# RLinf/RLinf

Measured on NVIDIA H100. Metric: env-steps/sec (rollout+update), higher is better.
Workload: dtype f32

## Files before the change

### include/rlinf_b200.h

```cpp
#ifndef RLINF_B200_H
#define RLINF_B200_H

#include <stdint.h>

#ifdef __cplusplus
extern "C" {
#endif

#define RB200_ABI_VERSION 2

#define RB200_OK 0
#define RB200_E_NULL (-1)
#define RB200_E_SHAPE (-2)
#define RB200_E_ARG (-3)
#define RB200_E_ALIGN (-4)
#define RB200_E_UNSUPPORTED (-5)

typedef void* rb200_stream_t;

int rb200_abi_version(void);
const char* rb200_strerror(int code);
int rb200_device_info(int* sm_count, int* cc_major, int* cc_minor);
uint64_t rb200_launch_count(void);

int rb200_loss_mask(const uint8_t* dones, uint8_t* mask, int64_t* mask_sum,
                    int nc, int B, int C, rb200_stream_t stream);

int rb200_gae(const float* rewards, const float* values, const uint8_t* dones,
              const uint8_t* loss_mask, float* adv, float* ret, double* stats,
              int T, int B, double gamma, double gae_lambda, rb200_stream_t stream);

int rb200_normalize(float* x, const double* stats, int64_t n_elems, float eps,
                    rb200_stream_t stream);

int rb200_grpo_scores(const float* rewards, const uint8_t* dones, float* scores,
                      int T, int B, rb200_stream_t stream);
int rb200_grpo_advantages(const float* scores, const uint8_t* loss_mask, float* adv,
                          int T, int B, int G, float eps, rb200_stream_t stream);

int rb200_gather_rows(const void* src, const int64_t* idx, void* dst, int64_t n_rows_out,
                      int64_t n_rows_src, int64_t row_bytes, rb200_stream_t stream);

enum { RB200_LOGPROB_TOKEN = 0, RB200_LOGPROB_ACTION = 1, RB200_LOGPROB_CHUNK = 2 };

enum {
  RB200_M_POLICY_LOSS = 0,
  RB200_M_POLICY_LOSS_ABS = 1,
  RB200_M_RATIO = 2,
  RB200_M_RATIO_ABS = 3,
  RB200_M_CLIPPED_RATIO = 4,
  RB200_M_DUAL_CLIPPED_RATIO = 5,
  RB200_M_APPROX_KL = 6,
  RB200_M_CLIP_FRACTION = 7,
  RB200_M_VALUE_LOSS = 8,
  RB200_M_VALUE_CLIP_RATIO = 9,
  RB200_M_EV_COUNT = 10,
  RB200_M_EV_RET_SUM = 11,
  RB200_M_EV_RET_SQ_SUM = 12,
  RB200_M_EV_ERR_SUM = 13,
  RB200_M_EV_ERR_SQ_SUM = 14,
  RB200_M_ENTROPY = 15,
  RB200_M_TOTAL_LOSS = 16,
  RB200_M_TOKEN_NUM = 17,
  RB200_NUM_METRICS = 24
};

typedef struct rb200_ppo_args {
  int64_t bsz;
  int32_t C, A;
  int32_t logprob_type;
  int32_t with_critic;
  const float* logprobs;
  const float* values;
  const float* entropy;
  const int64_t* idx;
  const float* old_logprobs;
  const float* advantages;
  const float* returns;
  const float* prev_values;
  const uint8_t* loss_mask;
  const int64_t* loss_mask_sum;
  int64_t mask_sum_row_mod;
  const double* adv_stats;
  float adv_norm_eps;
  double clip_ratio_low, clip_ratio_high;
  double clip_ratio_c;
  int32_t has_clip_log_ratio_min, has_clip_log_ratio_max;
  double clip_log_ratio_min, clip_log_ratio_max;
  double value_clip, huber_delta;
  int32_t max_episode_steps;
  int32_t critic_warmup;
  double entropy_bonus;
  double loss_scale;
  double* workspace;
  float* loss;
  float* metrics;
  float* d_logprobs;
  float* d_values;
  float* d_entropy;
} rb200_ppo_args;

int rb200_ppo_loss(const rb200_ppo_args* args, rb200_stream_t stream);

enum {
  RB200_DM_POLICY_LOSS = 0,
  RB200_DM_PROXIMAL_RATIO = 1,
  RB200_DM_CLIPPED_PROXIMAL_RATIO = 2,
  RB200_DM_CLIP_FRACTION = 3,
  RB200_DM_DUAL_CLIP_FRACTION = 4,
  RB200_DM_BEHAV_CLIP_FRACTION = 5,
  RB200_DM_PROXIMAL_APPROX_KL = 6,
  RB200_DM_BEHAV_APPROX_KL = 7,
  RB200_DM_VALUE_LOSS = 8,
  RB200_DM_VALUE_CLIP_RATIO = 9,
  RB200_DM_EV_COUNT = 10,
  RB200_DM_AVERAGE_VERSION = 15,
  RB200_DM_TOTAL_LOSS = 16,
  RB200_DM_TOKEN_NUM = 17,
  RB200_DM_CURRENT_VERSION = 18,
  RB200_DM_HAS_VERSION_METRICS = 19,
  RB200_DM_ENTROPY = 20
};
typedef struct rb200_dppo_args {
  rb200_ppo_args base;
  const float* proximal_logprobs;
  const float* versions;
  int32_t has_current_version;
  double current_version;
  int32_t has_behave_weight_threshold;
  double behave_weight_threshold;
} rb200_dppo_args;
int rb200_decoupled_ppo_loss(const rb200_dppo_args* args, rb200_stream_t stream);

typedef struct rb200_dppo_scalar_version_args {
  rb200_ppo_args base;
  const float* proximal_logprobs;
  double version;
  double current_version;
  int32_t has_behave_weight_threshold;
  double behave_weight_threshold;
} rb200_dppo_scalar_version_args;
int rb200_decoupled_ppo_loss_scalar_version(const rb200_dppo_scalar_version_args* args, rb200_stream_t stream);

enum { RB200_OM_POLICY_LOSS = 0, RB200_OM_OPD_REWARD = 1, RB200_OM_OPD_REVERSE_KL = 2, RB200_OM_TOTAL_LOSS = 16 };
int rb200_opd_loss(const float* logprobs, const float* advantages, const uint8_t* loss_mask,
                   const int64_t* loss_mask_sum, int64_t n_units, int tokens_per_unit, int max_episode_steps,
                   double loss_scale, double* workspace, float* loss ,
                   float* metrics , float* d_logprobs , rb200_stream_t stream);

enum { RB200_AGG_TOKEN_MEAN = 0, RB200_AGG_SEQ_MEAN_TOKEN_SUM = 1, RB200_AGG_SEQ_MEAN_TOKEN_MEAN = 2 };
enum {
  RB200_TM_POLICY_LOSS = 0,
  RB200_TM_POLICY_LOSS_ABS = 1,
  RB200_TM_RATIO = 2,
  RB200_TM_RATIO_ABS = 3,
  RB200_TM_CLIPPED_RATIO = 4,
  RB200_TM_DUAL_CLIPPED_RATIO = 5,
  RB200_TM_APPROX_KL = 6,
  RB200_TM_CLIP_FRACTION = 7,
  RB200_TM_ENTROPY_LOSS = 8,
  RB200_TM_KL_LOSS = 9,
  RB200_TM_FINAL_LOSS = 10,
  RB200_TM_ROLLOUT_TRAIN_KL = 11,
  RB200_TM_NUM = 16
};
typedef struct rb200_token_loss_args {
  int64_t bsz, L;
  const float* logprobs;            int64_t logprobs_stride;
  const float* old_logprobs;        int64_t old_logprobs_stride;
  const float* advantages;          int64_t advantages_stride;
  const uint8_t* loss_mask;         int64_t loss_mask_stride;
  const float* entropy;             int64_t entropy_stride;
  const float* ref_logprobs;        int64_t ref_logprobs_stride;
  const float* rollout_logprobs;    int64_t rollout_logprobs_stride;
  const float* recomputed_logprobs; int64_t recomputed_logprobs_stride;
  double clip_ratio_low, clip_ratio_high;
  double clip_ratio_c;
  double clip_log_ratio_min, clip_log_ratio_max;
  double entropy_bonus, kl_beta, importance_sampling_clip;
  int32_t has_clip_log_ratio_min, has_clip_log_ratio_max;
  int32_t agg;
  int32_t kl_mode;
  int32_t kl_order;
  int32_t importance_sampling_fix;
  int32_t fast_path_zero_loss_mask;
  int32_t reserved;
  void* workspace;
  int64_t workspace_bytes;
  float* loss;
  float* metrics;
  float* d_logprobs;
  float* d_entropy;
} rb200_token_loss_args;
int64_t rb200_token_loss_workspace_bytes(int64_t bsz, int64_t L);
int rb200_token_ppo_loss(const rb200_token_loss_args* args, rb200_stream_t stream);

enum {
  RB200_CM_VALUE_LOSS = 0,
  RB200_CM_VALUE_CLIP_RATIO = 1,
  RB200_CM_EV_COUNT = 2,
  RB200_CM_EV_RET_SUM = 3,
  RB200_CM_EV_RET_SQ_SUM = 4,
  RB200_CM_EV_ERR_SUM = 5,
  RB200_CM_EV_ERR_SQ_SUM = 6,
  RB200_CM_FINAL_VALUE_LOSS = 7,
  RB200_CM_NUM = 8
};
typedef struct rb200_token_critic_loss_args {
  int64_t bsz, L;
  const float* values;       int64_t values_stride;
  const float* returns;      int64_t returns_stride;
  const float* prev_values;  int64_t prev_values_stride;
  const uint8_t* loss_mask;  int64_t loss_mask_stride;
  double value_clip, huber_delta;
  void* workspace;
  int64_t workspace_bytes;
  float* loss;
  float* metrics;
  float* d_values;
} rb200_token_critic_loss_args;
int rb200_token_critic_loss(const rb200_token_critic_loss_args* args, rb200_stream_t stream);

int64_t rb200_value_head_workspace_bytes(int64_t n, int64_t H);
int rb200_value_head_fwd(const void* x, int64_t row_stride, const int64_t* rows, int64_t n, int64_t H, const void* w,
                         float* v, rb200_stream_t stream);
int rb200_value_head_bwd(const void* x, int64_t row_stride, const int64_t* rows, int64_t n, int64_t H, const float* g,
                         const void* w, const int64_t* inv_map, int64_t T, void* dx, void* dw, void* workspace,
                         int64_t workspace_bytes, rb200_stream_t stream);

int rb200_scale(float* x, int64_t n, float s, rb200_stream_t stream);
int rb200_scale_by(float* x, int64_t n, const float* s_dev, rb200_stream_t stream);

int rb200_grad_sqnorm(const float* grads, int64_t n, double* out_sq ,
                      rb200_stream_t stream);
int rb200_adamw_step(float* params, const float* grads, float* exp_avg, float* exp_avg_sq,
                     int64_t n, const int64_t* group_end_host, const double* group_lr_host,
                     int n_groups, double beta1, double beta2, double eps, double weight_decay,
                     float max_grad_norm, float grad_scale, const double* grad_sq ,
                     double* state , rb200_stream_t stream);
int rb200_adamw_step_dev(float* params, const float* grads, float* exp_avg, float* exp_avg_sq,
                         int64_t n, const int64_t* group_end_host, const double* group_lr_dev,
                         int n_groups, double beta1, double beta2, double eps, double weight_decay,
                         float max_grad_norm, float grad_scale, const double* grad_sq ,
                         double* state , rb200_stream_t stream);


typedef struct rb200_mlp_layout {
  int32_t obs_dim, act_dim , value_dim, hidden ;
  int64_t logstd;
  int64_t vw0, vb0, vw1, vb1, vw2, vb2, vw3;
  int64_t bw0, bb0, bw1, bb1, bw2, bb2;
  int64_t mw, mb;
  int64_t total;
} rb200_mlp_layout;

int rb200_mlp_layout_init(rb200_mlp_layout* L, int obs_dim, int act_dim, int value_dim, int hidden);

int64_t rb200_mlp_fwd_scratch_floats(const rb200_mlp_layout* L, int64_t n);

int64_t rb200_mlp_wsplit_floats(const rb200_mlp_layout* L);
int rb200_mlp_prepare_weights(const rb200_mlp_layout* L, const float* params, float* wsplit,
                              rb200_stream_t stream);

int rb200_mlp_forward(const rb200_mlp_layout* L, const float* params, const float* wsplit,
                      const float* states, const float* action, const int64_t* idx, int64_t n,
                      float* logprobs, float* entropy, float* values, float* acts, float* work,
                      const float* states_amax, rb200_stream_t stream);
int rb200_absmax(const float* x, int64_t rows, int cols, float* out, rb200_stream_t stream);

int rb200_mlp_backward(const rb200_mlp_layout* L, const float* params, const float* wsplit,
                       const float* states, const float* action, const int64_t* idx, int64_t n,
                       const float* d_logprobs, const float* d_entropy, const float* d_values,
                       const float* acts, float* work, float* grads, rb200_stream_t stream);

int rb200_mlp_sample(const rb200_mlp_layout* L, const float* params, const float* wsplit,
                     const float* states, const float* noise, uint64_t seed, uint64_t offset,
                     const uint64_t* counter_dev, int64_t n, float* action, float* logprobs, float* values,
                     float* work, rb200_stream_t stream);

int rb200_tc_gemm_h(const float* A, const float* B, float* C, int64_t M, int K, int mode, const float* amax,
                    float* work, rb200_stream_t stream);
int rb200_tc_wgrad_h(const float* Z, const float* H, float* dW, int64_t n, int IN, const float* amax,
                     rb200_stream_t stream);
int rb200_tc_dgrad_wgrad_h(const float* Z, const float* W, const float* H, float* dZprev, float* dW, float* colsum,
                           const float* amax_in, float* amax_out, int64_t n, int ngroups, float* work,
                           rb200_stream_t stream);

int rb200_debug_set_flags(int flags);

typedef struct rb200_rollout_args {
  float* states;
  float* actions;
  float* logprobs;
  float* values;
  float* rewards;
  uint8_t* terminations;
  uint8_t* truncations;
  uint8_t* dones;
  float* final_obs;
  float* final_values;
  const float* w_s;
  const float* w_a;
  int32_t* elapsed;
  const float* policy_noise;
  const float* env_noise;
  const uint64_t* counter_policy;
  const uint64_t* counter_env;
  float* episode_return;
  double* episode_acc;
  uint64_t seed_policy, seed_env, offset_policy;
  int32_t T, B;
  int32_t num_action_chunks;
  int32_t max_episode_steps, auto_reset;
  int32_t bootstrap_on_done;
  double gamma, p_term, noise_std, reward_noise_std;
} rb200_rollout_args;

int64_t rb200_rollout_fused_wt_floats(const rb200_mlp_layout* L);
int rb200_rollout_fused_supported(const rb200_mlp_layout* L, int B);
int rb200_rollout_fused_prepare(const rb200_mlp_layout* L, const float* params, float* wt, rb200_stream_t stream);
int rb200_rollout_fused(const rb200_mlp_layout* L, const float* params, const float* wt, const rb200_rollout_args* a,
                        rb200_stream_t stream);

int rb200_rollout_tc_supported(const rb200_mlp_layout* L, int num_action_chunks, int B);
int64_t rb200_rollout_tc_pack_bytes(const rb200_mlp_layout* L);
int rb200_rollout_tc_prepare(const rb200_mlp_layout* L, const float* params, const float* w_s, void* pack,
                             rb200_stream_t stream);
int rb200_rollout_tc(const rb200_mlp_layout* L, const float* params, const void* pack, const rb200_rollout_args* a,
                     rb200_stream_t stream);

int rb200_logits_logprob_entropy_fwd(const void* logits, int dtype, const int64_t* target, int64_t N, int64_t L,
                                     int64_t batch_stride, int64_t row_stride, int V, int v_lo, int v_hi,
                                     double inv_temperature, float* logprob, float* entropy, float* lse,
                                     rb200_stream_t stream);
int rb200_logits_logprob_entropy_bwd(const void* logits, int dtype, const int64_t* target, int64_t N, int64_t L,
                                     int64_t batch_stride, int64_t row_stride, int V, int v_lo, int v_hi,
                                     double inv_temperature, const float* lse, const float* entropy,
                                     const float* grad_logprob, const float* grad_entropy, void* dlogits,
                                     int64_t d_batch_stride, int64_t d_row_stride, rb200_stream_t stream);

int64_t rb200_lmhead_workspace_bytes(int64_t N, int64_t L, int H, int V, int v_lo, int v_hi, int64_t vocab_chunk);
int rb200_lmhead_logprob_entropy_fwd(const void* hidden, const void* weight, const int64_t* target, int64_t N, int64_t L,
                                     int64_t batch_stride, int64_t row_stride, int H, int V, int v_lo, int v_hi,
                                     double inv_temperature, float* logprob, float* entropy, float* lse,
                                     void* workspace, int64_t workspace_bytes, rb200_stream_t stream);
int rb200_lmhead_logprob_entropy_bwd(const void* hidden, const void* weight, const int64_t* target, int64_t N, int64_t L,
                                     int64_t batch_stride, int64_t row_stride, int H, int V, int v_lo, int v_hi,
                                     double inv_temperature, const float* lse, const float* entropy,
                                     const float* grad_logprob, const float* grad_entropy, void* d_hidden,
                                     void* d_weight, void* workspace, int64_t workspace_bytes, rb200_stream_t stream);

int64_t rb200_lmhead_vp_workspace_bytes(int64_t N, int64_t L, int H, int Vs, int64_t vocab_start, int v_lo, int v_hi,
                                        int64_t vocab_chunk);
int rb200_lmhead_vp_partials_fwd(const void* hidden, const void* weight_shard, const int64_t* target, int64_t N,
                                 int64_t L, int64_t batch_stride, int64_t row_stride, int H, int Vs,
                                 int64_t vocab_start, int v_lo, int v_hi, double inv_temperature, float* record,
                                 void* workspace, int64_t workspace_bytes, rb200_stream_t stream);
int rb200_lmhead_vp_logprob_entropy_bwd(const void* hidden, const void* weight_shard, const int64_t* target,
                                        int64_t N, int64_t L, int64_t batch_stride, int64_t row_stride, int H, int Vs,
                                        int64_t vocab_start, int v_lo, int v_hi, double inv_temperature,
                                        const float* lse, const float* entropy, const float* grad_logprob,
                                        const float* grad_entropy, float* d_hidden_partial, void* d_weight_shard,
                                        void* workspace, int64_t workspace_bytes, rb200_stream_t stream);
int rb200_logits_vp_partials_fwd(const void* logits, int dtype, const int64_t* target, int64_t N, int64_t L,
                                 int64_t batch_stride, int64_t row_stride, int Vs, int64_t vocab_start, int v_lo,
                                 int v_hi, double inv_temperature, float* record, rb200_stream_t stream);
int rb200_vp_combine(const float* records, int n_ranks, int64_t N, const int64_t* target, int vocab_shard, int v_lo,
                     int v_hi, float* logprob, float* entropy, float* lse, rb200_stream_t stream);

enum {
  RB200_RR_RESPONSE = 1,
  RB200_RR_PROMPT = 2,
  RB200_RR_BOUNDS = 4,
  RB200_RR_ORDER = 8,
  RB200_RR_MAX_PROMPT = 16,
  RB200_RR_CAPACITY = 32
};
int rb200_response_rows_plan(int layout, const int64_t* len0, const int64_t* len1, const int64_t* response_lengths,
                             int64_t bsz, int64_t S, int64_t L, int64_t T, int entropy_shift, const int64_t* tokens,
                             int64_t capacity, int64_t* rows, int64_t* targets, int64_t* cell_map,
                             int64_t* hidden_map, int64_t* cells, int64_t* status, rb200_stream_t stream);

enum {
  RB200_RR_SHARD = 64,
  RB200_RR_CP_ALIGN = 128
};
int rb200_response_rows_mp_plan(const int64_t* cu_seqlens_padded, const int64_t* seq_lengths,
                                const int64_t* response_lengths, const int64_t* responses, int64_t bsz, int64_t L,
                                int64_t T_c, int tp_size, int cp_size, int sequence_parallel, int tp_rank, int cp_rank,
                                int64_t capacity_c, int64_t capacity_k, int64_t* rows, int64_t* send, int64_t* unpad,
                                int64_t* slot_map, int64_t* targets, int64_t* cell_map, int64_t* cells,
                                int64_t* hidden_map, int64_t* status, rb200_stream_t stream);
int rb200_response_rows_mp_pack_grad(const float* dx, const int64_t* idx, void* out, int64_t n_out, int64_t H,
                                     rb200_stream_t stream);

int rb200_mlp_value(const rb200_mlp_layout* L, const float* params, const float* wsplit,
                    const float* states, int64_t n, float* values, float* work, rb200_stream_t stream);

int rb200_synth_env_step(const float* w_s, const float* w_a, const float* state, const float* action,
                         const float* noise, float* next_state, float* final_obs, float* reward,
                         uint8_t* term, uint8_t* trunc, uint8_t* done, int32_t* elapsed, float* z_scratch,
                         int B, int obs, int act, int max_episode_steps, int auto_reset, float p_term,
                         float noise_std, float reward_noise_std, uint64_t seed,
                         const uint64_t* counter_dev, rb200_stream_t stream);
int rb200_synth_env_chunk_step(const float* w_s, const float* w_a, const float* state, const float* chunk_actions,
                               const float* noise, float* next_state, float* final_obs, float* rewards,
                               uint8_t* term, uint8_t* trunc, uint8_t* done, int32_t* elapsed, float* scratch,
                               int B, int obs, int act, int C, int max_episode_steps, int auto_reset, float p_term,
                               float noise_std, float reward_noise_std, uint64_t seed, const uint64_t* counter_dev,
                               rb200_stream_t stream);
int rb200_bootstrap_rewards_ld(float* rewards, int ld_rewards, const float* final_values, int value_dim,
                               const uint8_t* flag, int ld_flag, int B, double gamma, rb200_stream_t stream);
int rb200_bootstrap_rewards(float* rewards, const float* final_values, const uint8_t* flag, int B,
                            int value_dim, double gamma, rb200_stream_t stream);
int rb200_counter_add(uint64_t* counter_dev, uint64_t inc, rb200_stream_t stream);

int rb200_mlp_mean(const rb200_mlp_layout* L, const float* params, const float* wsplit, const float* states,
                   int64_t n, float* action, float* logprobs, float* values, float* work, rb200_stream_t stream);
int rb200_episode_stats_step(const float* rewards, const uint8_t* done, int B, int C, int auto_reset, float* ret,
                             int32_t* len, uint8_t* prev_done, double* acc, float* episode, rb200_stream_t stream);
int rb200_episode_stats_reduce(const double* acc, int B, double* out, rb200_stream_t stream);
int rb200_train_episode_stats_step(const float* rewards, const uint8_t* done, int B, int C, int auto_reset,
                                   int last_step, float* ret, int32_t* len, double* acc, rb200_stream_t stream);

int rb200_reward_filter(const float* rewards, const uint8_t* loss_mask, uint8_t* out_mask, uint8_t* keep_env,
                        int nc, int B, int C, int group_size, float lower, float upper,
                        rb200_stream_t stream);

int rb200_kl_penalty(const float* logprob, const float* ref_logprob, float* out, float* d_logprob, int64_t n,
                     int mode, rb200_stream_t stream);

int rb200_masked_stats(const float* x, const uint8_t* mask, int64_t n, int64_t mask_div, double* out4,
                       rb200_stream_t stream);

int rb200_masked_moments(const float* x, const uint8_t* mask, int64_t n, double* out3 ,
                         rb200_stream_t stream);
int rb200_masked_normalize(const float* x, const uint8_t* mask, float* out, int64_t n, const double* stats3,
                           int mode, double eps, int unbiased, rb200_stream_t stream);
int rb200_raw_advantages(const float* scores , const uint8_t* loss_mask , float* adv ,
                         int L, int B, double* stats3, rb200_stream_t stream);
int rb200_reinpp_returns(const float* rewards , const uint8_t* loss_mask , const float* logprob,
                         const float* ref_logprob, float* ret , int L, int B, double kl_beta, int kl_mode,
                         double* stats3, rb200_stream_t stream);
int rb200_grpo_video_advantages(const float* rewards , const float* mask_f32, const uint8_t* mask_u8,
                                float* adv , int S, int B, int G, int mode, float eps, rb200_stream_t stream);
int rb200_grpo_dynamic_turn_advantages(const float* rewards , const int32_t* idx_to_traj ,
                                       float* turn_adv , int n, int num_trajectories, int G, int mode,
                                       float eps, rb200_stream_t stream);
int rb200_sub(const float* a, const float* b, float* out, int64_t n, rb200_stream_t stream);

#ifdef __cplusplus
}
#endif
#endif
```

### rlinf_b200/_lib.py

```python
from __future__ import annotations

import ctypes as C
import os
from typing import Optional

import torch

_PKG_DIR = os.path.dirname(os.path.abspath(__file__))
LIB_PATH = os.path.join(_PKG_DIR, "librlinf_b200.so")

c_void_p, c_int, c_int64, c_float, c_double, c_uint64 = C.c_void_p, C.c_int, C.c_int64, C.c_float, C.c_double, C.c_uint64

NUM_METRICS = 24
LOGPROB_TYPES = {"token_level": 0, "action_level": 1, "chunk_level": 2}

M_KEYS = {
    0: "actor/policy_loss", 1: "actor/policy_loss_abs", 2: "actor/ratio", 3: "actor/ratio_abs",
    4: "actor/clipped_ratio", 5: "actor/dual_cliped_ratio", 6: "actor/approx_kl", 7: "actor/clip_fraction",
    8: "critic/value_loss", 9: "critic/value_clip_ratio",
    10: "__sum__/_critic_explained_variance/count",
    11: "__sum__/_critic_explained_variance/returns_sum",
    12: "__sum__/_critic_explained_variance/returns_sq_sum",
    13: "__sum__/_critic_explained_variance/errors_sum",
    14: "__sum__/_critic_explained_variance/errors_sq_sum",
    15: "actor/entropy_loss", 16: "actor/total_loss", 17: "actor/token_num",
}
ACTOR_SLOTS = (0, 1, 2, 3, 4, 5, 6, 7)
CRITIC_SLOTS = (8, 9, 10, 11, 12, 13, 14)


class PpoArgs(C.Structure):
    _fields_ = [
        ("bsz", c_int64), ("C", C.c_int32), ("A", C.c_int32), ("logprob_type", C.c_int32), ("with_critic", C.c_int32),
        ("logprobs", c_void_p), ("values", c_void_p), ("entropy", c_void_p),
        ("idx", c_void_p), ("old_logprobs", c_void_p), ("advantages", c_void_p), ("returns", c_void_p),
        ("prev_values", c_void_p), ("loss_mask", c_void_p), ("loss_mask_sum", c_void_p),
        ("mask_sum_row_mod", c_int64),
        ("adv_stats", c_void_p), ("adv_norm_eps", c_float),
        ("clip_ratio_low", c_double), ("clip_ratio_high", c_double), ("clip_ratio_c", c_double),
        ("has_clip_log_ratio_min", C.c_int32), ("has_clip_log_ratio_max", C.c_int32),
        ("clip_log_ratio_min", c_double), ("clip_log_ratio_max", c_double),
        ("value_clip", c_double), ("huber_delta", c_double),
        ("max_episode_steps", C.c_int32), ("critic_warmup", C.c_int32),
        ("entropy_bonus", c_double), ("loss_scale", c_double),
        ("workspace", c_void_p),
        ("loss", c_void_p), ("metrics", c_void_p), ("d_logprobs", c_void_p), ("d_values", c_void_p),
        ("d_entropy", c_void_p),
    ]


class DppoArgs(C.Structure):
    _fields_ = [("base", PpoArgs), ("proximal_logprobs", c_void_p), ("versions", c_void_p),
                ("has_current_version", C.c_int32), ("current_version", c_double),
                ("has_behave_weight_threshold", C.c_int32), ("behave_weight_threshold", c_double)]


class DppoScalarVersionArgs(C.Structure):
    _fields_ = [("base", PpoArgs), ("proximal_logprobs", c_void_p), ("version", c_double),
                ("current_version", c_double), ("has_behave_weight_threshold", C.c_int32),
                ("behave_weight_threshold", c_double)]


class RolloutArgs(C.Structure):
    _fields_ = [(n, c_void_p) for n in (
        "states", "actions", "logprobs", "values", "rewards", "terminations", "truncations", "dones", "final_obs",
        "final_values", "w_s", "w_a", "elapsed", "policy_noise", "env_noise", "counter_policy", "counter_env",
        "episode_return", "episode_acc")] + [
        ("seed_policy", c_uint64), ("seed_env", c_uint64), ("offset_policy", c_uint64),
        ("T", C.c_int32), ("B", C.c_int32), ("num_action_chunks", C.c_int32), ("max_episode_steps", C.c_int32),
        ("auto_reset", C.c_int32), ("bootstrap_on_done", C.c_int32),
        ("gamma", c_double), ("p_term", c_double), ("noise_std", c_double), ("reward_noise_std", c_double),
    ]


DM_KEYS = {
    0: "actor/policy_loss", 1: "actor/proximal_ratio", 2: "actor/clipped_proximal_ratio", 3: "actor/clip_fraction",
    4: "actor/dual_clip_fraction", 5: "actor/behav_clip_fraction", 6: "actor/proximal_approx_kl",
    7: "actor/behav_approx_kl", 8: "critic/value_loss", 9: "critic/value_clip_ratio",
    10: "__sum__/_critic_explained_variance/count", 11: "__sum__/_critic_explained_variance/returns_sum",
    12: "__sum__/_critic_explained_variance/returns_sq_sum", 13: "__sum__/_critic_explained_variance/errors_sum",
    14: "__sum__/_critic_explained_variance/errors_sq_sum",
}
DM_ENTROPY = 20


AGG_MODES = {"token-mean": 0, "seq-mean-token-sum": 1, "seq-mean-token-mean": 2}
TM_NUM = 16
TM_KEYS = {
    0: "actor/policy_loss", 1: "actor/policy_loss_abs", 2: "actor/ratio", 3: "actor/ratio_abs",
    4: "actor/clipped_ratio", 5: "actor/dual_cliped_ratio", 6: "actor/approx_kl", 7: "actor/clip_fraction",
    8: "actor/entropy_loss", 9: "actor/kl_loss", 10: "actor/final_loss", 11: "actor/rollout_train_kl",
}


class TokenLossArgs(C.Structure):
    _fields_ = [("bsz", c_int64), ("L", c_int64)] + [
        f for name in ("logprobs", "old_logprobs", "advantages", "loss_mask", "entropy", "ref_logprobs",
                       "rollout_logprobs", "recomputed_logprobs") for f in ((name, c_void_p), (name + "_stride", c_int64))
    ] + [(n, c_double) for n in ("clip_ratio_low", "clip_ratio_high", "clip_ratio_c", "clip_log_ratio_min",
                                  "clip_log_ratio_max", "entropy_bonus", "kl_beta", "importance_sampling_clip")] + [
        (n, C.c_int32) for n in ("has_clip_log_ratio_min", "has_clip_log_ratio_max", "agg", "kl_mode", "kl_order",
                                 "importance_sampling_fix", "fast_path_zero_loss_mask", "reserved")] + [
        ("workspace", c_void_p), ("workspace_bytes", c_int64),
        ("loss", c_void_p), ("metrics", c_void_p), ("d_logprobs", c_void_p), ("d_entropy", c_void_p),
    ]


CM_NUM = 8
CM_KEYS = {
    0: "critic/value_loss", 1: "critic/value_clip_ratio",
    2: "__sum__/_critic_explained_variance/count",
    3: "__sum__/_critic_explained_variance/returns_sum",
    4: "__sum__/_critic_explained_variance/returns_sq_sum",
    5: "__sum__/_critic_explained_variance/errors_sum",
    6: "__sum__/_critic_explained_variance/errors_sq_sum",
    7: "critic/final_value_loss",
}


class TokenCriticLossArgs(C.Structure):
    _fields_ = [("bsz", c_int64), ("L", c_int64)] + [
        f for name in ("values", "returns", "prev_values", "loss_mask")
        for f in ((name, c_void_p), (name + "_stride", c_int64))
    ] + [("value_clip", c_double), ("huber_delta", c_double), ("workspace", c_void_p), ("workspace_bytes", c_int64),
         ("loss", c_void_p), ("metrics", c_void_p), ("d_values", c_void_p)]


class MlpLayout(C.Structure):
    _fields_ = [
        ("obs_dim", C.c_int32), ("act_dim", C.c_int32), ("value_dim", C.c_int32), ("hidden", C.c_int32),
        ("logstd", c_int64),
        ("vw0", c_int64), ("vb0", c_int64), ("vw1", c_int64), ("vb1", c_int64), ("vw2", c_int64), ("vb2", c_int64),
        ("vw3", c_int64),
        ("bw0", c_int64), ("bb0", c_int64), ("bw1", c_int64), ("bb1", c_int64), ("bw2", c_int64), ("bb2", c_int64),
        ("mw", c_int64), ("mb", c_int64), ("total", c_int64),
    ]


SIGNATURES = {
    "rb200_abi_version": (c_int, []),
    "rb200_strerror": (C.c_char_p, [c_int]),
    "rb200_device_info": (c_int, [C.POINTER(c_int)] * 3),
    "rb200_launch_count": (c_uint64, []),
    "rb200_loss_mask": (c_int, [c_void_p, c_void_p, c_void_p, c_int, c_int, c_int, c_void_p]),
    "rb200_gae": (c_int, [c_void_p] * 7 + [c_int, c_int, c_double, c_double, c_void_p]),
    "rb200_normalize": (c_int, [c_void_p, c_void_p, c_int64, c_float, c_void_p]),
    "rb200_grpo_scores": (c_int, [c_void_p, c_void_p, c_void_p, c_int, c_int, c_void_p]),
    "rb200_grpo_advantages": (c_int, [c_void_p, c_void_p, c_void_p, c_int, c_int, c_int, c_float, c_void_p]),
    "rb200_gather_rows": (c_int, [c_void_p, c_void_p, c_void_p, c_int64, c_int64, c_int64, c_void_p]),
    "rb200_ppo_loss": (c_int, [C.POINTER(PpoArgs), c_void_p]),
    "rb200_decoupled_ppo_loss": (c_int, [C.POINTER(DppoArgs), c_void_p]),
    "rb200_decoupled_ppo_loss_scalar_version": (c_int, [C.POINTER(DppoScalarVersionArgs), c_void_p]),
    "rb200_opd_loss": (c_int, [c_void_p] * 4 + [c_int64, c_int, c_int, c_double] + [c_void_p] * 5),
    "rb200_token_loss_workspace_bytes": (c_int64, [c_int64, c_int64]),
    "rb200_token_ppo_loss": (c_int, [C.POINTER(TokenLossArgs), c_void_p]),
    "rb200_scale": (c_int, [c_void_p, c_int64, c_float, c_void_p]),
    "rb200_scale_by": (c_int, [c_void_p, c_int64, c_void_p, c_void_p]),
    "rb200_grad_sqnorm": (c_int, [c_void_p, c_int64, c_void_p, c_void_p]),
    "rb200_adamw_step": (c_int, [c_void_p] * 4 + [c_int64, C.POINTER(c_int64), C.POINTER(c_double), c_int,
                                                  c_double, c_double, c_double, c_double, c_float, c_float,
                                                  c_void_p, c_void_p, c_void_p]),
    "rb200_adamw_step_dev": (c_int, [c_void_p] * 4 + [c_int64, C.POINTER(c_int64), c_void_p, c_int,
                                                      c_double, c_double, c_double, c_double, c_float, c_float,
                                                      c_void_p, c_void_p, c_void_p]),
    "rb200_mlp_layout_init": (c_int, [C.POINTER(MlpLayout), c_int, c_int, c_int, c_int]),
    "rb200_mlp_fwd_scratch_floats": (c_int64, [C.POINTER(MlpLayout), c_int64]),
    "rb200_mlp_wsplit_floats": (c_int64, [C.POINTER(MlpLayout)]),
    "rb200_mlp_prepare_weights": (c_int, [C.POINTER(MlpLayout), c_void_p, c_void_p, c_void_p]),
    "rb200_mlp_forward": (c_int, [C.POINTER(MlpLayout)] + [c_void_p] * 5 + [c_int64] + [c_void_p] * 7),
    "rb200_absmax": (c_int, [c_void_p, c_int64, c_int, c_void_p, c_void_p]),
    "rb200_mlp_backward": (c_int, [C.POINTER(MlpLayout)] + [c_void_p] * 5 + [c_int64] + [c_void_p] * 7),
    "rb200_mlp_sample": (c_int, [C.POINTER(MlpLayout)] + [c_void_p] * 4 + [c_uint64, c_uint64, c_void_p, c_int64] + [c_void_p] * 5),
    "rb200_tc_gemm_h": (c_int, [c_void_p, c_void_p, c_void_p, c_int64, c_int, c_int, c_void_p, c_void_p, c_void_p]),
    "rb200_tc_wgrad_h": (c_int, [c_void_p, c_void_p, c_void_p, c_int64, c_int, c_void_p, c_void_p]),
    "rb200_tc_dgrad_wgrad_h": (c_int, [c_void_p] * 8 + [c_int64, c_int, c_void_p, c_void_p]),
    "rb200_debug_set_flags": (c_int, [c_int]),
    "rb200_rollout_fused_wt_floats": (c_int64, [C.POINTER(MlpLayout)]),
    "rb200_rollout_fused_supported": (c_int, [C.POINTER(MlpLayout), c_int]),
    "rb200_rollout_fused_prepare": (c_int, [C.POINTER(MlpLayout), c_void_p, c_void_p, c_void_p]),
    "rb200_rollout_fused": (c_int, [C.POINTER(MlpLayout), c_void_p, c_void_p, C.POINTER(RolloutArgs), c_void_p]),
    "rb200_rollout_tc_supported": (c_int, [C.POINTER(MlpLayout), c_int, c_int]),
    "rb200_rollout_tc_pack_bytes": (c_int64, [C.POINTER(MlpLayout)]),
    "rb200_rollout_tc_prepare": (c_int, [C.POINTER(MlpLayout), c_void_p, c_void_p, c_void_p, c_void_p]),
    "rb200_rollout_tc": (c_int, [C.POINTER(MlpLayout), c_void_p, c_void_p, C.POINTER(RolloutArgs), c_void_p]),
    "rb200_logits_logprob_entropy_fwd": (c_int, [c_void_p, c_int, c_void_p, c_int64, c_int64, c_int64, c_int64, c_int,
                                                 c_int, c_int, c_double, c_void_p, c_void_p, c_void_p, c_void_p]),
    "rb200_logits_logprob_entropy_bwd": (c_int, [c_void_p, c_int, c_void_p, c_int64, c_int64, c_int64, c_int64, c_int,
                                                 c_int, c_int, c_double] + [c_void_p] * 5 + [c_int64, c_int64, c_void_p]),
    "rb200_lmhead_workspace_bytes": (c_int64, [c_int64, c_int64, c_int, c_int, c_int, c_int, c_int64]),
    "rb200_lmhead_logprob_entropy_fwd": (c_int, [c_void_p, c_void_p, c_void_p, c_int64, c_int64, c_int64, c_int64, c_int,
                                                 c_int, c_int, c_int, c_double] + [c_void_p] * 4 + [c_int64, c_void_p]),
    "rb200_lmhead_logprob_entropy_bwd": (c_int, [c_void_p, c_void_p, c_void_p, c_int64, c_int64, c_int64, c_int64, c_int,
                                                 c_int, c_int, c_int, c_double] + [c_void_p] * 7 + [c_int64, c_void_p]),
    "rb200_lmhead_vp_workspace_bytes": (c_int64, [c_int64, c_int64, c_int, c_int, c_int64, c_int, c_int, c_int64]),
    "rb200_lmhead_vp_partials_fwd": (c_int, [c_void_p, c_void_p, c_void_p, c_int64, c_int64, c_int64, c_int64, c_int,
                                             c_int, c_int64, c_int, c_int, c_double, c_void_p, c_void_p, c_int64,
                                             c_void_p]),
    "rb200_lmhead_vp_logprob_entropy_bwd": (c_int, [c_void_p, c_void_p, c_void_p, c_int64, c_int64, c_int64, c_int64,
                                                    c_int, c_int, c_int64, c_int, c_int, c_double] + [c_void_p] * 7
                                            + [c_int64, c_void_p]),
    "rb200_logits_vp_partials_fwd": (c_int, [c_void_p, c_int, c_void_p, c_int64, c_int64, c_int64, c_int64, c_int,
                                             c_int64, c_int, c_int, c_double, c_void_p, c_void_p]),
    "rb200_vp_combine": (c_int, [c_void_p, c_int, c_int64, c_void_p, c_int, c_int, c_int] + [c_void_p] * 4),
    "rb200_response_rows_plan": (c_int, [c_int, c_void_p, c_void_p, c_void_p, c_int64, c_int64, c_int64, c_int64,
                                         c_int, c_void_p, c_int64] + [c_void_p] * 6 + [c_void_p]),
    "rb200_response_rows_mp_plan": (c_int, [c_void_p] * 4 + [c_int64] * 3 + [c_int] * 5 + [c_int64] * 2
                                    + [c_void_p] * 9 + [c_void_p]),
    "rb200_response_rows_mp_pack_grad": (c_int, [c_void_p, c_void_p, c_void_p, c_int64, c_int64, c_void_p]),
    "rb200_token_critic_loss": (c_int, [C.POINTER(TokenCriticLossArgs), c_void_p]),
    "rb200_value_head_workspace_bytes": (c_int64, [c_int64, c_int64]),
    "rb200_value_head_fwd": (c_int, [c_void_p, c_int64, c_void_p, c_int64, c_int64, c_void_p, c_void_p, c_void_p]),
    "rb200_value_head_bwd": (c_int, [c_void_p, c_int64, c_void_p, c_int64, c_int64, c_void_p, c_void_p, c_void_p,
                                     c_int64, c_void_p, c_void_p, c_void_p, c_int64, c_void_p]),
    "rb200_mlp_value":(c_int, [C.POINTER(MlpLayout), c_void_p, c_void_p, c_void_p, c_int64, c_void_p, c_void_p, c_void_p]),
    "rb200_synth_env_step": (c_int, [c_void_p] * 13 + [c_int] * 5 + [c_float] * 3 + [c_uint64, c_void_p, c_void_p]),
    "rb200_synth_env_chunk_step": (c_int, [c_void_p] * 13 + [c_int] * 6 + [c_float] * 3 + [c_uint64, c_void_p, c_void_p]),
    "rb200_bootstrap_rewards_ld": (c_int, [c_void_p, c_int, c_void_p, c_int, c_void_p, c_int, c_int, c_double, c_void_p]),
    "rb200_bootstrap_rewards": (c_int, [c_void_p, c_void_p, c_void_p, c_int, c_int, c_double, c_void_p]),
    "rb200_reward_filter": (c_int, [c_void_p] * 4 + [c_int] * 4 + [c_float, c_float, c_void_p]),
    "rb200_kl_penalty": (c_int, [c_void_p] * 4 + [c_int64, c_int, c_void_p]),
    "rb200_masked_stats": (c_int, [c_void_p, c_void_p, c_int64, c_int64, c_void_p, c_void_p]),
    "rb200_counter_add": (c_int, [c_void_p, c_uint64, c_void_p]),
    "rb200_masked_moments": (c_int, [c_void_p, c_void_p, c_int64, c_void_p, c_void_p]),
    "rb200_masked_normalize": (c_int, [c_void_p, c_void_p, c_void_p, c_int64, c_void_p, c_int, c_double, c_int, c_void_p]),
    "rb200_raw_advantages": (c_int, [c_void_p, c_void_p, c_void_p, c_int, c_int, c_void_p, c_void_p]),
    "rb200_reinpp_returns": (c_int, [c_void_p] * 5 + [c_int, c_int, c_double, c_int, c_void_p, c_void_p]),
    "rb200_grpo_video_advantages": (c_int, [c_void_p] * 4 + [c_int, c_int, c_int, c_int, c_float, c_void_p]),
    "rb200_grpo_dynamic_turn_advantages": (c_int, [c_void_p] * 3 + [c_int, c_int, c_int, c_int, c_float, c_void_p]),
    "rb200_sub": (c_int, [c_void_p, c_void_p, c_void_p, c_int64, c_void_p]),
    "rb200_mlp_mean": (c_int, [C.POINTER(MlpLayout), c_void_p, c_void_p, c_void_p, c_int64] + [c_void_p] * 5),
    "rb200_episode_stats_step": (c_int, [c_void_p, c_void_p, c_int, c_int, c_int] + [c_void_p] * 6),
    "rb200_episode_stats_reduce": (c_int, [c_void_p, c_int, c_void_p, c_void_p]),
    "rb200_train_episode_stats_step": (c_int, [c_void_p, c_void_p] + [c_int] * 4 + [c_void_p] * 4),
}

_LIB: Optional[C.CDLL] = None


class Rb200Error(RuntimeError):
    pass


def load() -> C.CDLL:
    global _LIB
    if _LIB is not None:
        return _LIB
    if not os.path.exists(LIB_PATH):
        raise Rb200Error(
            f"{LIB_PATH} not found: build it with `python -m rlinf_b200.build` "
            "(nvcc, sm_90a). rlinf_b200 has no CPU or PyTorch fallback.")
    lib = C.CDLL(LIB_PATH)
    for name, (res, args) in SIGNATURES.items():
        fn = getattr(lib, name)
        fn.restype = res
        fn.argtypes = args
    _LIB = lib
    return lib


def check(code: int, what: str = "") -> None:
    if code == 0:
        return
    msg = load().rb200_strerror(code).decode()
    if code < 0:
        raise ValueError(f"rlinf_b200 {what}: {msg} (code {code})")
    raise Rb200Error(f"rlinf_b200 {what}: CUDA error {code}: {msg}")


def ptr(t: Optional[torch.Tensor]):
    if t is None:
        return None
    if not t.is_cuda:
        raise Rb200Error("rlinf_b200 kernels take CUDA tensors; move inputs with to_device() first")
    if not t.is_contiguous():
        raise Rb200Error("rlinf_b200 kernels take contiguous tensors")
    return c_void_p(t.data_ptr())


def stream_ptr(device=None):
    return c_void_p(torch.cuda.current_stream(device).cuda_stream)


def default_device() -> torch.device:
    if not torch.cuda.is_available():
        raise Rb200Error("rlinf_b200 needs a CUDA device (H100, sm_90a); there is no CPU fallback")
    return torch.device("cuda", torch.cuda.current_device())


def to_device(t: Optional[torch.Tensor], device=None, dtype=None) -> Optional[torch.Tensor]:
    if t is None:
        return None
    device = device or default_device()
    if t.device != device:
        t = t.to(device, non_blocking=True)
    if dtype is not None and t.dtype != dtype:
        t = t.to(dtype)
    return t.contiguous()


def as_u8(t: Optional[torch.Tensor]) -> Optional[torch.Tensor]:
    if t is None:
        return None
    if t.dtype == torch.bool:
        return t.view(torch.uint8)
    if t.dtype != torch.uint8:
        return (t != 0).view(torch.uint8)
    return t
```

### rlinf_b200/actor.py

```python
from __future__ import annotations

from typing import Optional

import numpy as np
import torch
import torch.distributed as dist

from . import _lib as L
from . import dist_utils as D
from . import ops
from .algorithms import calculate_adv_and_returns
from .config import wrap
from .lr_scheduler import LRSchedule
from .policy import FlatAdamW, MLPPolicy

EV_KEY = "critic/explained_variance"
_T_PLUS_ONE_KEYS = ("dones", "terminations", "truncations", "prev_values")


def process_nested_dict_for_adv(nested, rollout_epoch):
    out = {}
    for k, v in nested.items():
        if isinstance(v, dict):
            out[k] = process_nested_dict_for_adv(v, rollout_epoch)
        elif isinstance(v, torch.Tensor):
            x = v.reshape(rollout_epoch, -1, *v.shape[1:]).transpose(0, 1)
            out[k] = x.reshape(x.shape[0], -1, *x.shape[3:])
    return out


def process_nested_dict_for_train(nested, shuffle_id):
    out = {}
    for k, v in nested.items():
        if v is None:
            out[k] = None
        elif isinstance(v, dict):
            out[k] = process_nested_dict_for_train(v, shuffle_id)
        elif isinstance(v, torch.Tensor):
            if k in _T_PLUS_ONE_KEYS:
                v = v[:-1]
            flat = v.reshape(-1, *v.shape[2:])
            if any(s == 0 for s in flat.stride()) and flat.numel() > 1:
                flat = flat.contiguous()
            as_bool = flat.dtype == torch.bool
            src = flat.contiguous()
            res = ops.gather_rows(src.view(torch.uint8) if as_bool else src, shuffle_id)
            out[k] = res.view(torch.bool) if as_bool else res
    return out


class EmbodiedActor:
    def __init__(self, cfg, policy: Optional[MLPPolicy] = None, rank: Optional[int] = None,
                 world_size: Optional[int] = None, process_group=None):
        self.cfg = wrap(cfg)
        self.pg = process_group
        self._dist = dist.is_available() and dist.is_initialized()
        self._rank = rank if rank is not None else (dist.get_rank() if self._dist else 0)
        self._world_size = world_size if world_size is not None else (dist.get_world_size() if self._dist else 1)
        m = self.cfg.actor.model
        self.device = L.default_device()
        self.model = policy or MLPPolicy(m.obs_dim, m.action_dim, m.get("num_action_chunks", 1),
                                         add_value_head=m.get("add_value_head", True), device=self.device,
                                         seed=self.cfg.actor.seed)
        o = self.cfg.actor.optim
        self.optimizer = FlatAdamW(self.model, lr=o.lr, value_lr=o.get("value_lr", o.lr),
                                   betas=(o.get("adam_beta1", 0.9), o.get("adam_beta2", 0.999)),
                                   eps=o.get("adam_eps", 1e-8), weight_decay=o.get("weight_decay", 1e-2),
                                   clip_grad=o.get("clip_grad", 1.0))
        self.optimizer_steps = 0
        self.critic_warmup_steps = int(o.get("critic_warmup_steps", 0) or 0) if self.model.value_dim > 0 else 0
        self._with_critic = self.cfg.algorithm.adv_type == "gae"
        self._set_frozen_groups()
        self.lr_schedule = LRSchedule(o, base_lr=o.lr)
        self.optimizer.lr_scale = self.lr_schedule.multiplier()
        self.rollout_batch: dict = {}
        self._perm_cache: dict = {}
        self.version = 0
        self._graph_update = self.cfg.actor.get("cuda_graph_update", False)
        self._graph_multi_rank = bool(self.cfg.actor.get("cuda_graph_multi_rank", False))
        self._capture_nccl = bool(self.cfg.actor.get("cuda_graph_capture_nccl", True))
        self._static_batch: dict = {}
        self._step_graphs: dict = {}
        self._train_calls = 0
        self._states_amax = torch.zeros(4 + m.obs_dim if m.obs_dim <= 256 else 1, dtype=torch.float32,
                                        device=self.device) if m.obs_dim % 32 == 0 else None

    def recv_rollout_trajectories(self, batch: dict) -> None:
        def to_dev(d):
            return {k: (to_dev(v) if isinstance(v, dict) else L.to_device(v, self.device)) for k, v in d.items()
                    if v is not None}

        self.rollout_batch = self._process_received_rollout_batch(to_dev(batch))

    def _process_received_rollout_batch(self, rollout_batch: dict) -> dict:
        cfg = self.cfg
        rollout_epoch = cfg.env.train.get("rollout_epoch", 1)
        if rollout_epoch != 1:
            rollout_batch = process_nested_dict_for_adv(rollout_batch, rollout_epoch)
        if not cfg.env.train.auto_reset and not cfg.env.train.get("ignore_terminations", False):
            loss_mask, loss_mask_sum = ops.loss_mask(rollout_batch["dones"])
            if cfg.algorithm.reward_type == "chunk_level":
                loss_mask = loss_mask.any(dim=-1, keepdim=True)
                loss_mask_sum = loss_mask_sum[..., -1:]
            rollout_batch["loss_mask"] = loss_mask
            rollout_batch["loss_mask_sum"] = loss_mask_sum
        if cfg.algorithm.get("filter_rewards", False):
            rollout_batch["loss_mask"] = ops.reward_filter(
                rollout_batch["rewards"], rollout_batch.get("loss_mask", None), cfg.algorithm.group_size,
                cfg.algorithm.rewards_lower_bound, cfg.algorithm.rewards_upper_bound)
        return rollout_batch

    def compute_advantages_and_returns(self) -> dict:
        cfg, rb = self.cfg, self.rollout_batch
        kwargs = {
            "task_type": cfg.runner.task_type, "adv_type": cfg.algorithm.adv_type, "rewards": rb["rewards"],
            "dones": rb["dones"], "values": rb.get("prev_values", None), "prev_logprobs": rb.get("prev_logprobs", None),
            "teacher_logprobs": None, "num_action_chunks": cfg.actor.model.get("num_action_chunks", 1),
            "gamma": cfg.algorithm.get("gamma", 1), "gae_lambda": cfg.algorithm.get("gae_lambda", 1),
            "group_size": cfg.algorithm.get("group_size", 8), "reward_type": cfg.algorithm.reward_type,
            "loss_mask": rb.get("loss_mask", None), "loss_mask_sum": rb.get("loss_mask_sum", None),
            "advantage_mode": cfg.algorithm.get("advantage_mode", None),
        }
        rb.update(calculate_adv_and_returns(**kwargs))
        if not cfg.runner.get("rollout_metrics", True):
            return {}
        from .metric_utils import compute_rollout_metrics

        return compute_rollout_metrics(rb, self._world_size, self.pg)

    def _shuffle_id(self, n: int) -> torch.Tensor:
        key = (n, self.cfg.actor.seed + self._rank)
        if key not in self._perm_cache:
            g = torch.Generator()
            g.manual_seed(D.shuffle_seed(self.cfg.actor.seed, self._rank))
            self._perm_cache[key] = torch.randperm(n, generator=g).to(self.device)
        return self._perm_cache[key]

    def run_training(self) -> dict:
        cfg = self.cfg
        rb = self.rollout_batch
        rollout_size = rb["prev_logprobs"].shape[0] * rb["prev_logprobs"].shape[1]
        shuffle_id = self._shuffle_id(rollout_size)
        batch = process_nested_dict_for_train(rb, shuffle_id)
        self.rollout_batch = batch
        mbs = cfg.actor.micro_batch_size
        batch_size_per_rank, self.gradient_accumulation, n_global = D.per_rank_batch(
            cfg.actor.global_batch_size, self._world_size, mbs, rollout_size)
        update_epoch = cfg.algorithm.get("update_epoch", 1)
        n_steps = update_epoch * n_global
        n_micro = n_steps * self.gradient_accumulation
        metric_rows = torch.zeros(n_micro, L.NUM_METRICS, dtype=torch.float32, device=self.device)
        step_rows = torch.zeros(n_steps, 4, dtype=torch.float64, device=self.device)
        lr_rows = []
        mi = si = 0
        use_graph = self._graph_update
        if use_graph == "auto":
            use_graph = batch_size_per_rank <= 65536
        if self._world_size > 1 and not self._graph_multi_rank:
            use_graph = False
        graphed = bool(use_graph) and self._train_calls > 0
        self._train_calls += 1
        if graphed:
            batch = self._persist_batch(batch)
            self.rollout_batch = batch
        if self._states_amax is not None:
            ops.absmax(batch["forward_inputs"]["states"], out=self._states_amax)
        for _ in range(update_epoch):
            for gb in range(n_global):
                if graphed:
                    lr_rows.append(self._graphed_step(batch, gb, batch_size_per_rank, mbs,
                                                      metric_rows[mi: mi + self.gradient_accumulation], step_rows[si]))
                    mi += self.gradient_accumulation
                    si += 1
                    continue
                self.optimizer.zero_grad()
                for k in range(self.gradient_accumulation):
                    lo = gb * batch_size_per_rank + k * mbs
                    self.train_micro_batch(batch, lo, lo + mbs, metric_rows[mi])
                    mi += 1
                grad_norm_state, lr_list = self.optimizer_step()
                step_rows[si].copy_(grad_norm_state)
                lr_rows.append(lr_list)
                si += 1
        self.optimizer.lr_scale = self.lr_schedule.step()
        self.optimizer.zero_grad()
        return self._reduce_metrics(metric_rows, step_rows, lr_rows)

    def _persist_batch(self, batch: dict, prefix: str = "") -> dict:
        out = {}
        for k, v in batch.items():
            key = prefix + k
            if isinstance(v, dict):
                out[k] = self._persist_batch(v, key + "/")
            elif isinstance(v, torch.Tensor):
                buf = self._static_batch.get(key)
                if buf is None or buf.shape != v.shape or buf.dtype != v.dtype:
                    buf = torch.empty_like(v)
                    self._static_batch[key] = buf
                    self._step_graphs.clear()
                buf.copy_(v)
                out[k] = buf
            else:
                out[k] = v
        return out

    def _graphed_step(self, batch, gb, batch_size_per_rank, mbs, metric_out, state_out):
        warm = self.optimizer_steps < self.critic_warmup_steps
        accum = self.gradient_accumulation
        key = (gb, warm, accum, mbs, batch_size_per_rank, self._world_size)
        self.optimizer.sync_lr_table()
        entry = self._step_graphs.get(key)
        if entry is None:
            stage_m = torch.zeros(accum, L.NUM_METRICS, dtype=torch.float32, device=self.device)
            stage_s = torch.zeros(4, dtype=torch.float64, device=self.device)
            scale = 1.0 / self._world_size

            def fwd_bwd():
                self.optimizer.zero_grad()
                for k in range(accum):
                    lo = gb * batch_size_per_rank + k * mbs
                    self.train_micro_batch(batch, lo, lo + mbs, stage_m[k])

            def opt():
                self.optimizer.step(grad_scale=scale)
                stage_s.copy_(self.optimizer.state)

            graphs = None
            if self._world_size > 1 and self._capture_nccl:
                try:
                    torch.cuda.synchronize()
                    self.model.mark_params_changed()
                    g_all = torch.cuda.CUDAGraph()
                    with torch.cuda.graph(g_all):
                        fwd_bwd()
                        dist.all_reduce(self.model.flat_grads, op=dist.ReduceOp.SUM, group=self.pg)
                        opt()
                    graphs = (g_all, None)
                except Exception as e:
                    self._capture_nccl = False
                    self._capture_nccl_error = repr(e)
                    torch.cuda.synchronize()
            if graphs is None:
                torch.cuda.synchronize()
                self.model.mark_params_changed()
                g_a = torch.cuda.CUDAGraph()
                with torch.cuda.graph(g_a):
                    fwd_bwd()
                g_b = torch.cuda.CUDAGraph()
                with torch.cuda.graph(g_b, pool=g_a.pool()):
                    opt()
                graphs = (g_a, g_b)
            entry = (graphs, stage_m, stage_s)
            self._step_graphs[key] = entry
        (g_a, g_b), stage_m, stage_s = entry
        g_a.replay()
        self.optimizer_steps += 1
        if g_b is not None:
            D.allreduce_flat_grads(self.model.flat_grads, self._world_size, self.pg)
            g_b.replay()
        self.model.mark_params_changed()
        metric_out.copy_(stage_m)
        state_out.copy_(stage_s)
        return self._after_optimizer_step()

    def train_micro_batch(self, batch, lo, hi, metric_out) -> None:
        cfg = self.cfg
        fi = batch["forward_inputs"]
        with_critic = self._with_critic
        ent_bonus = float(cfg.algorithm.get("entropy_bonus", 0) or 0)
        warm = self.optimizer_steps < self.critic_warmup_steps
        out = self.model.forward_train(fi["states"][lo:hi], fi["action"][lo:hi], compute_entropy=ent_bonus > 0,
                                       compute_values=with_critic, states_amax=self._states_amax)
        A = cfg.actor.model.get("action_dim", 7)
        Cc = out["logprobs"].shape[1] // A
        U = 1 if cfg.algorithm.logprob_type == "chunk_level" else Cc
        n = hi - lo

        def unit(key):
            t = batch.get(key)
            return None if t is None else t[lo:hi].reshape(n, U)

        loss, metrics, d_lp, d_v, d_e = ops.ppo_loss(
            logprobs=out["logprobs"], values=out.get("values") if with_critic else None,
            entropy=out.get("entropy"), old_logprobs=batch["prev_logprobs"][lo:hi].reshape(n, Cc * A),
            advantages=unit("advantages"), returns=unit("returns") if with_critic else None,
            prev_values=unit("prev_values") if with_critic else None, loss_mask=unit("loss_mask"),
            loss_mask_sum=unit("loss_mask_sum"), C_chunks=Cc, A_dim=A, logprob_type=cfg.algorithm.logprob_type,
            clip_ratio_low=cfg.algorithm.clip_ratio_low, clip_ratio_high=cfg.algorithm.clip_ratio_high,
            value_clip=cfg.algorithm.get("value_clip", None), huber_delta=cfg.algorithm.get("huber_delta", None),
            max_episode_steps=cfg.env.train.max_episode_steps if batch.get("loss_mask_sum") is not None else None,
            critic_warmup=warm, entropy_bonus=ent_bonus, loss_scale=1.0 / self.gradient_accumulation)
        metric_out.copy_(metrics)
        self.model.backward(d_lp, d_v if with_critic else None, d_e)

    def _set_frozen_groups(self):
        frozen = set()
        if self.critic_warmup_steps > 0:
            frozen.add("actor")
        if not self._with_critic:
            frozen.add("critic")
        self.optimizer.frozen = frozen

    def _after_optimizer_step(self):
        if self.critic_warmup_steps > 0:
            lr_list = [0.0 for _ in self.optimizer.lr_list()]
            if self.optimizer_steps >= self.critic_warmup_steps:
                self.critic_warmup_steps = 0
                self._set_frozen_groups()
                self.optimizer.reset_state(carry_grads=True)
                self.lr_schedule = LRSchedule(self.cfg.actor.optim, base_lr=self.cfg.actor.optim.lr)
                self.optimizer.lr_scale = self.lr_schedule.multiplier()
            return lr_list
        return self.optimizer.lr_list()

    def state_dict(self) -> dict:
        return {"optimizer": self.optimizer.state_dict(), "optimizer_steps": int(self.optimizer_steps),
                "critic_warmup_steps": int(self.critic_warmup_steps),
                "lr_last_epoch": int(self.lr_schedule.last_epoch), "lr_scale": float(self.optimizer.lr_scale)}

    def load_state_dict(self, sd: dict) -> None:
        self.optimizer.load_state_dict(sd["optimizer"])
        self.optimizer_steps = int(sd["optimizer_steps"])
        self.critic_warmup_steps = int(sd["critic_warmup_steps"])
        self._set_frozen_groups()
        self.lr_schedule.last_epoch = int(sd["lr_last_epoch"])
        self.optimizer.lr_scale = float(sd["lr_scale"])
        self.model.mark_params_changed()

    def optimizer_step(self):
        self.optimizer_steps += 1
        scale = D.allreduce_flat_grads(self.model.flat_grads, self._world_size, self.pg)
        self.optimizer.step(grad_scale=scale)
        state = self.optimizer.state.clone()
        return state, self._after_optimizer_step()

    def _reduce_metrics(self, metric_rows, step_rows, lr_rows) -> dict:
        with_critic = self.cfg.algorithm.adv_type == "gae"
        mean_vec = metric_rows.mean(dim=0)
        ev_sum = metric_rows[:, 10:15].sum(dim=0)
        grad_norm = step_rows[:, 1].mean().to(torch.float32)
        packed = D.reduce_metric_pack(mean_vec, ev_sum, grad_norm, self._world_size, self.pg)
        host = packed.tolist()
        out = {}
        slots = L.ACTOR_SLOTS + ((8, 9) if with_critic else ()) + (15, 16)
        for s in slots:
            out[L.M_KEYS[s]] = host[s]
        out["actor/grad_norm"] = host[-1]
        out["actor/lr"] = float(np.mean([r[0] for r in lr_rows]))
        second = [r[1] for r in lr_rows if len(r) > 1]
        if second:
            out["critic/lr"] = float(np.mean(second))
        if with_critic:
            cnt, rs, rss, es, ess = host[L.NUM_METRICS: L.NUM_METRICS + 5]
            ev = float("nan")
            if cnt >= 2:
                rc = rss - rs * rs / cnt
                ec = ess - es * es / cnt
                if rc == rc and rc != 0 and ec == ec:
                    ev = 1 - ec / rc
            out[EV_KEY] = ev
        return out

    def sync_model_to_rollout(self, rollout_params: Optional[torch.Tensor] = None, src: int = 0):
        if rollout_params is not None and rollout_params.data_ptr() != self.model.flat_params.data_ptr():
            rollout_params.copy_(self.model.flat_params)
        if self.cfg.runner.get("broadcast_params", True):
            from .weight_sync import broadcast_flat

            self.rollout_version = broadcast_flat(self.model, self.version, src, self.pg)
        self.model.mark_params_changed()
```

### rlinf_b200/csrc/mlp.cu

```cuda
#include <curand_kernel.h>

#include "common.cuh"
#include "sgemm.cuh"
#include "tc_gemm.cuh"

namespace {

using namespace rb::gemm;

__global__ void __launch_bounds__(256) absmax_kernel(const float4* __restrict__ x, int64_t n4, int cols4, int cols,
                                                     float* __restrict__ out) {
  __shared__ unsigned int s_col[256];
  __shared__ unsigned int s_all;
  for (int c = threadIdx.x; c < 256; c += blockDim.x) s_col[c] = 0u;
  if (threadIdx.x == 0) s_all = 0u;
  __syncthreads();
  float4 m = make_float4(0.f, 0.f, 0.f, 0.f);
  for (int64_t i = (int64_t)blockIdx.x * blockDim.x + threadIdx.x; i < n4; i += (int64_t)gridDim.x * blockDim.x) {
    const float4 v = __ldg(x + i);
    m.x = fmaxf(m.x, fabsf(v.x)); m.y = fmaxf(m.y, fabsf(v.y)); m.z = fmaxf(m.z, fabsf(v.z)); m.w = fmaxf(m.w, fabsf(v.w));
  }
  atomicMax(&s_all, __float_as_uint(fmaxf(fmaxf(m.x, m.y), fmaxf(m.z, m.w))));
  if (cols) {
    const int c0 = 4 * (threadIdx.x % cols4);
    atomicMax(&s_col[c0], __float_as_uint(m.x)); atomicMax(&s_col[c0 + 1], __float_as_uint(m.y));
    atomicMax(&s_col[c0 + 2], __float_as_uint(m.z)); atomicMax(&s_col[c0 + 3], __float_as_uint(m.w));
  }
  __syncthreads();
  if (threadIdx.x == 0 && s_all) atomicMax(reinterpret_cast<unsigned int*>(out), s_all);
  for (int c = threadIdx.x; c < cols; c += blockDim.x)
    if (s_col[c]) atomicMax(reinterpret_cast<unsigned int*>(out + 4 + c), s_col[c]);
}

constexpr int kH = 256;
constexpr int kMaxAct = 32;
constexpr int kMaxVal = 8;
constexpr float kHalfLog2Pi = 0.91893853320467274178f;

struct HeadFwdArgs {
  const float* h3;
  const float* g3;
  const float* mw;
  const float* mb;
  const float* logstd;
  const float* vw3;
  const float* action;
  const int64_t* idx;
  const float* noise;
  uint64_t seed, offset;
  const uint64_t* counter;
  int sample_mode;
  float* mean_out;
  float* action_out;
  float* logprobs;
  float* entropy;
  float* values;
  int64_t n;
  int act, vdim;
};

__global__ void __launch_bounds__(256) head_fwd_kernel(HeadFwdArgs p) {
  extern __shared__ float sm[];
  float* s_mw = sm;
  float* s_vw = sm + p.act * kH;
  for (int i = threadIdx.x; i < p.act * kH; i += blockDim.x) s_mw[i] = p.mw[i];
  if (p.g3 && p.values)
    for (int i = threadIdx.x; i < p.vdim * kH; i += blockDim.x) s_vw[i] = p.vw3[i];
  __syncthreads();
  const int lane = threadIdx.x & 31, warp = threadIdx.x >> 5, nwarp = blockDim.x >> 5;
  const bool want_v = p.g3 && p.values;
  const int64_t row_stride = (int64_t)gridDim.x * nwarp;
  float4 nh0 = make_float4(0.f, 0.f, 0.f, 0.f), nh1 = nh0, ng0 = nh0, ng1 = nh0;
  auto fetch = [&](int64_t r) {
    if (r < p.n) {
      nh0 = __ldg(reinterpret_cast<const float4*>(p.h3 + r * kH + lane * 4));
      nh1 = __ldg(reinterpret_cast<const float4*>(p.h3 + r * kH + 128 + lane * 4));
      if (want_v) {
        ng0 = __ldg(reinterpret_cast<const float4*>(p.g3 + r * kH + lane * 4));
        ng1 = __ldg(reinterpret_cast<const float4*>(p.g3 + r * kH + 128 + lane * 4));
      }
    }
  };
  fetch((int64_t)blockIdx.x * nwarp + warp);
  for (int64_t row = (int64_t)blockIdx.x * nwarp + warp; row < p.n; row += row_stride) {
    const float4 h0 = nh0, h1 = nh1, pg0 = ng0, pg1 = ng1;
    fetch(row + row_stride);
    float my_mean = 0.f;
    for (int a = 0; a < p.act; ++a) {
      const float4 w0 = *reinterpret_cast<const float4*>(s_mw + a * kH + lane * 4);
      const float4 w1 = *reinterpret_cast<const float4*>(s_mw + a * kH + 128 + lane * 4);
      float s = h0.x * w0.x + h0.y * w0.y + h0.z * w0.z + h0.w * w0.w + h1.x * w1.x + h1.y * w1.y + h1.z * w1.z +
                h1.w * w1.w;
      s = rb::warp_sum(s);
      if (lane == a) my_mean = s + p.mb[a];
    }
    if (lane < p.act) {
      const float ls = p.logstd[lane];
      const float sd = expf(ls);
      float x;
      if (p.sample_mode == 2) {
        x = my_mean;
        p.action_out[row * p.act + lane] = x;
      } else if (p.sample_mode) {
        float z;
        if (p.noise) {
          z = p.noise[row * p.act + lane];
        } else {
          curandStatePhilox4_32_10_t st;
          curand_init(p.seed, (unsigned long long)(row * p.act + lane), p.offset + 4ull * (p.counter ? p.counter[0] : 0ull), &st);
          z = curand_normal(&st);
        }
        x = my_mean + sd * z;
        p.action_out[row * p.act + lane] = x;
      } else {
        const int64_t src = p.idx ? p.idx[row] : row;
        x = p.action[src * p.act + lane];
      }
      const float d = x - my_mean;
      const float var = sd * sd;
      if (p.logprobs) p.logprobs[row * p.act + lane] = -(d * d) / (2.0f * var) - logf(sd) - kHalfLog2Pi;
      if (p.entropy) p.entropy[row * p.act + lane] = 0.5f + kHalfLog2Pi + logf(sd);
      if (p.mean_out) p.mean_out[row * p.act + lane] = my_mean;
    }
    if (want_v) {
      const float4 g0 = pg0, g1 = pg1;
      for (int c = 0; c < p.vdim; ++c) {
        const float4 w0 = *reinterpret_cast<const float4*>(s_vw + c * kH + lane * 4);
        const float4 w1 = *reinterpret_cast<const float4*>(s_vw + c * kH + 128 + lane * 4);
        float s = g0.x * w0.x + g0.y * w0.y + g0.z * w0.z + g0.w * w0.w + g1.x * w1.x + g1.y * w1.y + g1.z * w1.z +
                  g1.w * w1.w;
        s = rb::warp_sum(s);
        if (lane == 0) p.values[row * p.vdim + c] = s;
      }
    }
  }
}

struct HeadBwdArgs {
  const float* h3;
  const float* g3;
  const float* mean;
  const float* mw;
  const float* logstd;
  const float* vw3;
  const float* action;
  const int64_t* idx;
  const float* d_logprobs;
  const float* d_entropy;
  const float* d_values;
  float* dz3;
  float* dy3;
  float* g_mw;
  float* g_mb;
  float* g_logstd;
  float* g_vw3;
  float* g_b2;
  float* g_vb2;
  float* amax_dz3;
  float* amax_dy3;
  float* part;
  int64_t n;
  int act, vdim;
};

template <bool REG>
__global__ void __launch_bounds__(256) head_bwd_kernel(HeadBwdArgs p) {
  extern __shared__ float sm[];
  const int lane = threadIdx.x & 31, warp = threadIdx.x >> 5, nwarp = blockDim.x >> 5;
  const int acc_len = (p.act + p.vdim) * kH + 64 + 2 * kH;
  float* s_mw = sm;
  float* s_vw = s_mw + p.act * kH;
  float* acc0 = s_vw + p.vdim * kH;
  float* a_mw = acc0 + warp * acc_len;
  float* a_vw = a_mw + p.act * kH;
  float* a_mb = a_vw + p.vdim * kH;
  float* a_ls = a_mb + 32;
  float* a_b2 = a_ls + 32;
  float* a_vb2 = a_b2 + kH;
  const bool has_v = p.d_values != nullptr;
  for (int i = threadIdx.x; i < p.act * kH; i += blockDim.x) s_mw[i] = p.mw[i];
  for (int i = threadIdx.x; i < p.vdim * kH; i += blockDim.x) s_vw[i] = has_v ? p.vw3[i] : 0.f;
  for (int i = threadIdx.x; i < nwarp * acc_len; i += blockDim.x) acc0[i] = 0.f;
  __syncthreads();
  float cb[8] = {0.f, 0.f, 0.f, 0.f, 0.f, 0.f, 0.f, 0.f}, cv[8] = {0.f, 0.f, 0.f, 0.f, 0.f, 0.f, 0.f, 0.f};
  float mz = 0.f, my = 0.f;
  float rm[REG ? 8 : 1][8], rv[REG ? 2 : 1][8];
#pragma unroll
  for (int a = 0; a < (REG ? 8 : 1); ++a)
#pragma unroll
    for (int j = 0; j < 8; ++j) rm[a][j] = 0.f;
#pragma unroll
  for (int c = 0; c < (REG ? 2 : 1); ++c)
#pragma unroll
    for (int j = 0; j < 8; ++j) rv[c][j] = 0.f;
  struct RowIn {
    float4 h0, h1, g0, g1;
    float x, mu, dlp, den, dv0, dv1;
  };
  auto load_row = [&](int64_t row) -> RowIn {
    RowIn r;
    r.h0 = r.h1 = r.g0 = r.g1 = make_float4(0.f, 0.f, 0.f, 0.f);
    r.x = r.mu = r.dlp = r.den = r.dv0 = r.dv1 = 0.f;
    if (row < p.n) {
      r.h0 = __ldg(reinterpret_cast<const float4*>(p.h3 + row * kH + lane * 4));
      r.h1 = __ldg(reinterpret_cast<const float4*>(p.h3 + row * kH + 128 + lane * 4));
      if (has_v) {
        r.g0 = __ldg(reinterpret_cast<const float4*>(p.g3 + row * kH + lane * 4));
        r.g1 = __ldg(reinterpret_cast<const float4*>(p.g3 + row * kH + 128 + lane * 4));
        if (REG) {
          r.dv0 = __ldg(p.d_values + row * p.vdim);
          if (p.vdim > 1) r.dv1 = __ldg(p.d_values + row * p.vdim + 1);
        }
      }
      if (lane < p.act) {
        const int64_t src = p.idx ? p.idx[row] : row;
        r.x = __ldg(p.action + src * p.act + lane);
        r.mu = __ldg(p.mean + row * p.act + lane);
        r.dlp = __ldg(p.d_logprobs + row * p.act + lane);
        if (p.d_entropy) r.den = __ldg(p.d_entropy + row * p.act + lane);
      }
    }
    return r;
  };
  const int64_t row_stride = (int64_t)gridDim.x * nwarp;
  const int64_t row_first = (int64_t)blockIdx.x * nwarp + warp;
  const float sd_l = lane < p.act ? expf(p.logstd[lane]) : 1.f;
  const float var_l = sd_l * sd_l;
  RowIn nxt0 = load_row(row_first), nxt1 = load_row(row_first + row_stride);
  for (int64_t row = row_first; row < p.n; row += row_stride) {
    const RowIn cur = nxt0;
    nxt0 = nxt1;
    nxt1 = load_row(row + 2 * row_stride);
    const float4 h0 = cur.h0, h1 = cur.h1;
    float dmu = 0.f;
    if (lane < p.act) {
      const float d = cur.x - cur.mu;
      dmu = cur.dlp * d / var_l;
      const float dls = cur.dlp * (d * d / var_l - 1.0f) + cur.den;
      atomicAdd(&a_mb[lane], dmu);
      atomicAdd(&a_ls[lane], dls);
    }
    float4 dh0 = make_float4(0.f, 0.f, 0.f, 0.f), dh1 = dh0;
#pragma unroll
    for (int a = 0; a < (REG ? 8 : kMaxAct); ++a) {
      if (a >= p.act) break;
      const float g = __shfl_sync(0xffffffffu, dmu, a);
      const float4 w0 = *reinterpret_cast<const float4*>(s_mw + a * kH + lane * 4);
      const float4 w1 = *reinterpret_cast<const float4*>(s_mw + a * kH + 128 + lane * 4);
      dh0.x += g * w0.x; dh0.y += g * w0.y; dh0.z += g * w0.z; dh0.w += g * w0.w;
      dh1.x += g * w1.x; dh1.y += g * w1.y; dh1.z += g * w1.z; dh1.w += g * w1.w;
      if (REG) {
        const int ar = a < 8 ? a : 0;
        rm[ar][0] += g * h0.x; rm[ar][1] += g * h0.y; rm[ar][2] += g * h0.z; rm[ar][3] += g * h0.w;
        rm[ar][4] += g * h1.x; rm[ar][5] += g * h1.y; rm[ar][6] += g * h1.z; rm[ar][7] += g * h1.w;
        continue;
      }
      float* am = a_mw + a * kH;
      atomicAdd(&am[lane * 4 + 0], g * h0.x); atomicAdd(&am[lane * 4 + 1], g * h0.y);
      atomicAdd(&am[lane * 4 + 2], g * h0.z); atomicAdd(&am[lane * 4 + 3], g * h0.w);
      atomicAdd(&am[128 + lane * 4 + 0], g * h1.x); atomicAdd(&am[128 + lane * 4 + 1], g * h1.y);
      atomicAdd(&am[128 + lane * 4 + 2], g * h1.z); atomicAdd(&am[128 + lane * 4 + 3], g * h1.w);
    }
    float4 o0, o1;
    o0.x = dh0.x * (1.f - h0.x * h0.x); o0.y = dh0.y * (1.f - h0.y * h0.y);
    o0.z = dh0.z * (1.f - h0.z * h0.z); o0.w = dh0.w * (1.f - h0.w * h0.w);
    o1.x = dh1.x * (1.f - h1.x * h1.x); o1.y = dh1.y * (1.f - h1.y * h1.y);
    o1.z = dh1.z * (1.f - h1.z * h1.z); o1.w = dh1.w * (1.f - h1.w * h1.w);
    *reinterpret_cast<float4*>(p.dz3 + row * kH + lane * 4) = o0;
    *reinterpret_cast<float4*>(p.dz3 + row * kH + 128 + lane * 4) = o1;
    cb[0] += o0.x; cb[1] += o0.y; cb[2] += o0.z; cb[3] += o0.w;
    cb[4] += o1.x; cb[5] += o1.y; cb[6] += o1.z; cb[7] += o1.w;
    mz = fmaxf(mz, fmaxf(fmaxf(fmaxf(fabsf(o0.x), fabsf(o0.y)), fmaxf(fabsf(o0.z), fabsf(o0.w))),
                         fmaxf(fmaxf(fabsf(o1.x), fabsf(o1.y)), fmaxf(fabsf(o1.z), fabsf(o1.w)))));

    if (has_v) {
      const float4 g0 = cur.g0, g1 = cur.g1;
      float4 dg0 = make_float4(0.f, 0.f, 0.f, 0.f), dg1 = dg0;
#pragma unroll
      for (int c = 0; c < (REG ? 2 : kMaxVal); ++c) {
        if (c >= p.vdim) break;
        const float g = REG ? (c == 0 ? cur.dv0 : cur.dv1) : p.d_values[row * p.vdim + c];
        const float4 w0 = *reinterpret_cast<const float4*>(s_vw + c * kH + lane * 4);
        const float4 w1 = *reinterpret_cast<const float4*>(s_vw + c * kH + 128 + lane * 4);
        dg0.x += g * w0.x; dg0.y += g * w0.y; dg0.z += g * w0.z; dg0.w += g * w0.w;
        dg1.x += g * w1.x; dg1.y += g * w1.y; dg1.z += g * w1.z; dg1.w += g * w1.w;
        if (REG) {
          const int cr = c < 2 ? c : 0;
          rv[cr][0] += g * g0.x; rv[cr][1] += g * g0.y; rv[cr][2] += g * g0.z; rv[cr][3] += g * g0.w;
          rv[cr][4] += g * g1.x; rv[cr][5] += g * g1.y; rv[cr][6] += g * g1.z; rv[cr][7] += g * g1.w;
          continue;
        }
        float* av = a_vw + c * kH;
        atomicAdd(&av[lane * 4 + 0], g * g0.x); atomicAdd(&av[lane * 4 + 1], g * g0.y);
        atomicAdd(&av[lane * 4 + 2], g * g0.z); atomicAdd(&av[lane * 4 + 3], g * g0.w);
        atomicAdd(&av[128 + lane * 4 + 0], g * g1.x); atomicAdd(&av[128 + lane * 4 + 1], g * g1.y);
        atomicAdd(&av[128 + lane * 4 + 2], g * g1.z); atomicAdd(&av[128 + lane * 4 + 3], g * g1.w);
      }
      float4 q0, q1;
      q0.x = dg0.x * (1.f - g0.x * g0.x); q0.y = dg0.y * (1.f - g0.y * g0.y);
      q0.z = dg0.z * (1.f - g0.z * g0.z); q0.w = dg0.w * (1.f - g0.w * g0.w);
      q1.x = dg1.x * (1.f - g1.x * g1.x); q1.y = dg1.y * (1.f - g1.y * g1.y);
      q1.z = dg1.z * (1.f - g1.z * g1.z); q1.w = dg1.w * (1.f - g1.w * g1.w);
      *reinterpret_cast<float4*>(p.dy3 + row * kH + lane * 4) = q0;
      *reinterpret_cast<float4*>(p.dy3 + row * kH + 128 + lane * 4) = q1;
      cv[0] += q0.x; cv[1] += q0.y; cv[2] += q0.z; cv[3] += q0.w;
      cv[4] += q1.x; cv[5] += q1.y; cv[6] += q1.z; cv[7] += q1.w;
      my = fmaxf(my, fmaxf(fmaxf(fmaxf(fabsf(q0.x), fabsf(q0.y)), fmaxf(fabsf(q0.z), fabsf(q0.w))),
                           fmaxf(fmaxf(fabsf(q1.x), fabsf(q1.y)), fmaxf(fabsf(q1.z), fabsf(q1.w)))));
    }
  }
  if (p.amax_dz3 != nullptr) {
#pragma unroll
    for (int o = 16; o > 0; o >>= 1) {
      mz = fmaxf(mz, __shfl_xor_sync(0xffffffffu, mz, o));
      my = fmaxf(my, __shfl_xor_sync(0xffffffffu, my, o));
    }
    if (lane == 0) {
      if (mz > 0.f) atomicMax(reinterpret_cast<unsigned int*>(p.amax_dz3), __float_as_uint(mz));
      if (has_v && my > 0.f && p.amax_dy3) atomicMax(reinterpret_cast<unsigned int*>(p.amax_dy3), __float_as_uint(my));
    }
  }
#pragma unroll
  for (int j = 0; j < 4; ++j) {
    atomicAdd(&a_b2[lane * 4 + j], cb[j]);
    atomicAdd(&a_b2[128 + lane * 4 + j], cb[4 + j]);
    if (has_v) {
      atomicAdd(&a_vb2[lane * 4 + j], cv[j]);
      atomicAdd(&a_vb2[128 + lane * 4 + j], cv[4 + j]);
    }
  }
  if (REG) {
#pragma unroll
    for (int a = 0; a < 8; ++a) {
      if (a >= p.act) break;
      float* am = a_mw + a * kH;
#pragma unroll
      for (int j = 0; j < 4; ++j) {
        atomicAdd(&am[lane * 4 + j], rm[a][j]);
        atomicAdd(&am[128 + lane * 4 + j], rm[a][4 + j]);
      }
    }
    if (has_v) {
#pragma unroll
      for (int c = 0; c < 2; ++c) {
        if (c >= p.vdim) break;
        float* av = a_vw + c * kH;
#pragma unroll
        for (int j = 0; j < 4; ++j) {
          atomicAdd(&av[lane * 4 + j], rv[c][j]);
          atomicAdd(&av[128 + lane * 4 + j], rv[c][4 + j]);
        }
      }
    }
  }
  __syncthreads();
  for (int i = threadIdx.x; i < acc_len; i += blockDim.x) {
    float s = 0.f;
    for (int w = 0; w < nwarp; ++w) s += acc0[w * acc_len + i];
    p.part[(size_t)blockIdx.x * acc_len + i] = s;
  }
}

int head_grid(int64_t n) {
  int64_t blocks = (n + 7) / 8;
  const int64_t cap = (int64_t)rb::sm_count() * 4;
  if (blocks > cap) blocks = cap;
  return (int)(blocks < 1 ? 1 : blocks);
}

struct TowerW {
  const float *w0, *b0, *w1, *b1, *w2, *b2;
};
int layer_forward(const float* in, const int64_t* idx, int64_t n, int in_dim, const float* w, const float* b,
                  float* out, cudaStream_t st) {
  GemmArgs g{};
  g.M = n; g.N = kH; g.ldc = kH; g.k_per_split = 1 << 30;
  g.A = in; g.lda = in_dim; g.a_rows = idx; g.B = w; g.ldb = in_dim; g.K = in_dim; g.bias = b; g.C = out;
  return launch_gemm<A_KCONTIG, B_KCONTIG, EPI_BIAS_TANH>(g, 1, st);
}


struct TowerWH {
  const float *w0f, *w1f, *w2f;
  const float *w1d, *w2d;
};

struct TowerIO {
  TowerW w;
  TowerWH wh;
  float *H1, *H2, *H3;
  float *g_w0, *g_b0, *g_w1, *g_b1, *g_w2, *g_b2;
  const float* dZ3;
  float *tA, *tB;
  float* amax;
};

bool layer0_on_tc(const int64_t* idx, int in_dim) { return idx == nullptr && in_dim % rb::tc::BK == 0; }

float* x_amax_slot(const rb200_mlp_layout* L, float* buf, int64_t n) { return buf + 6 * n * kH + n * L->act_dim; }
int64_t x_amax_floats(int cols) { return cols <= 256 ? 4 + cols : 1; }

int publish_absmax(const float* X, int64_t rows, int cols, float* out, cudaStream_t st) {
  if (reinterpret_cast<uintptr_t>(X) & 15) return RB200_E_ALIGN;
  if (cols % 4 != 0) return RB200_E_SHAPE;
  cudaError_t ce = cudaMemsetAsync(out, 0, sizeof(float) * x_amax_floats(cols), st);
  if (ce != cudaSuccess) return (int)ce;
  const int cols4 = cols / 4, col_out = cols <= 256 ? cols : 0;
  const int threads = col_out ? cols4 * (256 / cols4) : 256;
  const int64_t n4 = rows * cols4;
  int64_t blocks = (n4 + threads - 1) / threads;
  const int64_t cap = (int64_t)rb::sm_count() * 4;
  if (blocks > cap) blocks = cap;
  absmax_kernel<<<(int)(blocks < 1 ? 1 : blocks), threads, 0, st>>>(reinterpret_cast<const float4*>(X), n4,
                                                                    col_out ? cols4 : 1, col_out, out);
  rb::count_launch();
  ce = cudaPeekAtLastError();
  return ce == cudaSuccess ? 0 : (int)ce;
}

int towers_forward_h(const float* X, const int64_t* idx, int64_t n, int in_dim, TowerIO* t, int nt, float* x_amax,
                     const float* x_amax_in, cudaStream_t st) {
  int e;
  const bool l0_tc = layer0_on_tc(idx, in_dim);
  rb::tch::GemmLaunch g[2];
  auto gemm = [&](int K) {
    return K <= rb::tc::BN ? rb::tch::forward(g, nt, n, K, rb::tc::EPI_BIAS_TANH, st)
                           : rb::tch::launch(g, nt, n, K, rb::tc::EPI_BIAS_TANH, 0, st);
  };
  if (l0_tc) {
    if (x_amax_in) {
      cudaError_t ce = cudaMemcpyAsync(x_amax, x_amax_in, sizeof(float) * x_amax_floats(in_dim), cudaMemcpyDeviceToDevice, st);
      if (ce != cudaSuccess) return (int)ce;
    } else if ((e = publish_absmax(X, n, in_dim, x_amax, st))) {
      return e;
    }
    for (int i = 0; i < nt; ++i) g[i] = rb::tch::GemmLaunch{X, t[i].wh.w0f, t[i].H1, t[i].w.b0, nullptr, nullptr, nullptr, nullptr, x_amax};
    if ((e = gemm(in_dim))) return e;
  } else {
    for (int i = 0; i < nt; ++i)
      if ((e = layer_forward(X, idx, n, in_dim, t[i].w.w0, t[i].w.b0, t[i].H1, st))) return e;
  }
  for (int i = 0; i < nt; ++i) g[i] = rb::tch::GemmLaunch{t[i].H1, t[i].wh.w1f, t[i].H2, t[i].w.b1, nullptr, nullptr, nullptr, nullptr};
  if ((e = gemm(kH))) return e;
  for (int i = 0; i < nt; ++i) g[i] = rb::tch::GemmLaunch{t[i].H2, t[i].wh.w2f, t[i].H3, t[i].w.b2, nullptr, nullptr, nullptr, nullptr};
  return gemm(kH);
}

int simt_wgrad_chunks(int64_t n, int64_t* rows_per_chunk) {
  int64_t chunks = (n + 255) / 256;
  const int64_t cap = rb::sm_count() / 2 > 1 ? rb::sm_count() / 2 : 1;
  if (chunks > cap) chunks = cap;
  const int64_t rows = (n + chunks - 1) / chunks;
  *rows_per_chunk = rows;
  return (int)((n + rows - 1) / rows);
}

int towers_backward_h(const float* X, const int64_t* idx, int64_t n, int in_dim, TowerIO* t, int nt,
                      const float* x_amax, cudaStream_t st) {
  int e;
  rb::tch::WgradLaunch w[2];
  rb::tch::BackwardLaunch b[2];
  for (int i = 0; i < nt; ++i)
    b[i] = rb::tch::BackwardLaunch{t[i].dZ3, t[i].wh.w2d, t[i].H2, t[i].tA, t[i].g_w2, t[i].g_b1, t[i].amax, t[i].amax + 1,
                                   t[i].tB};
  if ((e = rb::tch::dgrad_wgrad(b, nt, n, st))) return e;
  for (int i = 0; i < nt; ++i)
    b[i] = rb::tch::BackwardLaunch{t[i].tA, t[i].wh.w1d, t[i].H1, t[i].tB, t[i].g_w1, t[i].g_b0, t[i].amax + 1, t[i].amax + 2,
                                   const_cast<float*>(t[i].dZ3)};
  if ((e = rb::tch::dgrad_wgrad(b, nt, n, st))) return e;
  if (layer0_on_tc(idx, in_dim) && in_dim <= 256) {
    for (int i = 0; i < nt; ++i) w[i] = rb::tch::WgradLaunch{t[i].tB, X, t[i].g_w0, t[i].amax + 2, x_amax + 4};
    return rb::tch::wgrad(w, nt, n, in_dim, st);
  }
  int64_t rows = 0;
  const int chunks = simt_wgrad_chunks(n, &rows);
  const int64_t slab = (int64_t)kH * in_dim;
  float* part = rb::partials_scratch(chunks * slab);
  if (!part) return RB200_E_UNSUPPORTED;
  for (int i = 0; i < nt; ++i) {
    GemmArgs a{};
    a.A = t[i].tB; a.lda = kH; a.B = X; a.ldb = in_dim; a.b_rows = idx; a.C = part; a.c_split_stride = slab;
    a.ldc = in_dim; a.M = kH; a.N = in_dim; a.K = n; a.k_per_split = rows;
    if ((e = launch_gemm<A_MCONTIG, B_NCONTIG, EPI_STORE>(a, chunks, st))) return e;
    rb::tch::SlotSums ss{};
    ss.count = 1;
    ss.nslab = chunks;
    ss.stride = slab;
    ss.part[0] = part;
    ss.out[0] = t[i].g_w0;
    ss.len[0] = (int)slab;
    if ((e = rb::tch::sum_slots(ss, st))) return e;
  }
  return 0;
}

}

extern "C" int rb200_mlp_layout_init(rb200_mlp_layout* L, int obs_dim, int act_dim, int value_dim, int hidden) {
  if (!L) return RB200_E_NULL;
  if (obs_dim <= 0 || act_dim <= 0 || value_dim < 0) return RB200_E_SHAPE;
  if (hidden != kH || act_dim > kMaxAct || value_dim > kMaxVal) return RB200_E_UNSUPPORTED;
  L->obs_dim = obs_dim; L->act_dim = act_dim; L->value_dim = value_dim; L->hidden = hidden;
  int64_t o = 0;
  auto take = [&](int64_t n) { o = (o + 3) & ~int64_t(3); const int64_t at = o; o += n; return at; };
  L->logstd = take(act_dim);
  L->vw0 = take((int64_t)hidden * obs_dim); L->vb0 = take(hidden);
  L->vw1 = take((int64_t)hidden * hidden); L->vb1 = take(hidden);
  L->vw2 = take((int64_t)hidden * hidden); L->vb2 = take(hidden);
  L->vw3 = take((int64_t)value_dim * hidden);
  L->bw0 = take((int64_t)hidden * obs_dim); L->bb0 = take(hidden);
  L->bw1 = take((int64_t)hidden * hidden); L->bb1 = take(hidden);
  L->bw2 = take((int64_t)hidden * hidden); L->bb2 = take(hidden);
  L->mw = take((int64_t)act_dim * hidden); L->mb = take(act_dim);
  L->total = (o + 3) & ~int64_t(3);
  const int64_t sms = rb::sm_count(), head = 4 * sms * ((act_dim + value_dim) * hidden + 64 + 2 * hidden);
  const int64_t wg = sms / 2 * hidden * (obs_dim > hidden ? obs_dim : hidden) + sms * hidden;
  if (!rb::partials_scratch(head > wg ? head : wg)) (void)cudaGetLastError();
  return RB200_OK;
}

static inline int64_t act_floats(int64_t n) { return n * kH; }

extern "C" int64_t rb200_mlp_fwd_scratch_floats(const rb200_mlp_layout* L, int64_t n) {
  if (!L || n <= 0) return 0;
  return 6 * act_floats(n) + n * L->act_dim + 64 + 256;
}

static inline int64_t wsplit_tower_floats(int obs) { return (int64_t)kH * obs + 4ll * kH * kH; }

extern "C" int64_t rb200_mlp_wsplit_floats(const rb200_mlp_layout* L) {
  if (!L) return 0;
  return 2 * wsplit_tower_floats(L->obs_dim);
}

static int check_layout(const rb200_mlp_layout* L) {
  if (!L) return RB200_E_NULL;
  if (L->hidden != kH || L->act_dim <= 0 || L->act_dim > kMaxAct || L->value_dim < 0 || L->value_dim > kMaxVal)
    return RB200_E_UNSUPPORTED;
  return RB200_OK;
}

namespace {
TowerW tower_w(const rb200_mlp_layout* L, const float* P, bool value) {
  TowerW w;
  if (value) {
    w.w0 = P + L->vw0; w.b0 = P + L->vb0; w.w1 = P + L->vw1; w.b1 = P + L->vb1; w.w2 = P + L->vw2; w.b2 = P + L->vb2;
  } else {
    w.w0 = P + L->bw0; w.b0 = P + L->bb0; w.w1 = P + L->bw1; w.b1 = P + L->bb1; w.w2 = P + L->bw2; w.b2 = P + L->bb2;
  }
  return w;
}
TowerWH tower_wh(const rb200_mlp_layout* L, const float* ws, bool value) {
  const int64_t n0 = (int64_t)kH * L->obs_dim, nn = (int64_t)kH * kH;
  const float* b = ws + (value ? 0 : wsplit_tower_floats(L->obs_dim));
  TowerWH t;
  t.w0f = b;
  t.w1f = b + n0;
  t.w2f = b + n0 + nn;
  t.w1d = b + n0 + 2 * nn;
  t.w2d = b + n0 + 3 * nn;
  return t;
}

TowerIO tower_io(const rb200_mlp_layout* L, const float* P, const float* wsplit, bool value, float* h, int64_t n) {
  TowerIO t{};
  t.w = tower_w(L, P, value);
  t.wh = tower_wh(L, wsplit, value);
  t.H1 = h;
  t.H2 = h + act_floats(n);
  t.H3 = h + 2 * act_floats(n);
  return t;
}

int forward_towers(const rb200_mlp_layout* L, const float* P, const float* wsplit, const float* states,
                   const int64_t* idx, int64_t n, bool policy, bool value, float* buf, const float* x_amax_in,
                   cudaStream_t st) {
  TowerIO t[2];
  int nt = 0;
  if (policy) t[nt++] = tower_io(L, P, wsplit, false, buf, n);
  if (value) t[nt++] = tower_io(L, P, wsplit, true, buf + 3 * act_floats(n), n);
  return towers_forward_h(states, idx, n, L->obs_dim, t, nt, x_amax_slot(L, buf, n), x_amax_in, st);
}

int head_forward(const rb200_mlp_layout* L, const float* P, const float* buf, int64_t n, float* values, HeadFwdArgs h,
                 cudaStream_t st) {
  h.h3 = buf + 2 * act_floats(n); h.g3 = values ? buf + 5 * act_floats(n) : nullptr;
  h.mw = P + L->mw; h.mb = P + L->mb; h.logstd = P + L->logstd; h.vw3 = P + L->vw3;
  h.values = values; h.n = n; h.act = L->act_dim; h.vdim = L->value_dim;
  const size_t smem = sizeof(float) * (size_t)(L->act_dim + (values ? L->value_dim : 0)) * kH;
  head_fwd_kernel<<<head_grid(n), 256, smem, st>>>(h);
  rb::count_launch();
  RB_RETURN_LAUNCH();
}
}

extern "C" int rb200_mlp_prepare_weights(const rb200_mlp_layout* L, const float* params, float* wsplit,
                                         rb200_stream_t stream) {
  int e = check_layout(L);
  if (e) return e;
  if (!params || !wsplit) return RB200_E_NULL;
  rb::tch::SplitSpec sp[6];
  int cnt = 0;
  for (int v = 0; v < 2; ++v) {
    if (v == 0 && L->value_dim == 0) continue;
    const TowerW w = tower_w(L, params, v == 0);
    const TowerWH t = tower_wh(L, wsplit, v == 0);
    const int64_t n0 = (int64_t)kH * L->obs_dim, nn = (int64_t)kH * kH;
    if (L->obs_dim % rb::tc::BK == 0)
      sp[cnt++] = rb::tch::SplitSpec{w.w0, const_cast<float*>(t.w0f), nullptr, n0};
    sp[cnt++] = rb::tch::SplitSpec{w.w1, const_cast<float*>(t.w1f), const_cast<float*>(t.w1d), nn};
    sp[cnt++] = rb::tch::SplitSpec{w.w2, const_cast<float*>(t.w2f), const_cast<float*>(t.w2d), nn};
  }
  return rb::tch::split_weights(sp, cnt, rb::as_stream(stream));
}

extern "C" int rb200_mlp_forward(const rb200_mlp_layout* L, const float* params, const float* wsplit,
                                 const float* states, const float* action, const int64_t* idx, int64_t n,
                                 float* logprobs, float* entropy, float* values, float* acts, float* work,
                                 const float* states_amax, rb200_stream_t stream) {
  int e = check_layout(L);
  if (e) return e;
  if (!params || !wsplit || !states || !action || !logprobs || !acts || !work) return RB200_E_NULL;
  if (n <= 0) return RB200_E_SHAPE;
  if (values && L->value_dim == 0) return RB200_E_SHAPE;
  cudaStream_t st = rb::as_stream(stream);
  if ((e = forward_towers(L, params, wsplit, states, idx, n, true, values != nullptr, acts, states_amax, st))) return e;
  HeadFwdArgs h{};
  h.action = action; h.idx = idx; h.sample_mode = 0; h.mean_out = acts + 6 * act_floats(n); h.logprobs = logprobs;
  h.entropy = entropy;
  return head_forward(L, params, acts, n, values, h, st);
}

extern "C" int rb200_mlp_backward(const rb200_mlp_layout* L, const float* params, const float* wsplit,
                                  const float* states, const float* action, const int64_t* idx, int64_t n,
                                  const float* d_logprobs, const float* d_entropy, const float* d_values,
                                  const float* acts, float* work, float* grads, rb200_stream_t stream) {
  int e = check_layout(L);
  if (e) return e;
  if (!params || !wsplit || !states || !action || !d_logprobs || !acts || !work || !grads) return RB200_E_NULL;
  if (n <= 0) return RB200_E_SHAPE;
  cudaStream_t st = rb::as_stream(stream);
  const int64_t PF = act_floats(n);
  const float *H3 = acts + 2 * PF, *G3 = acts + 5 * PF, *mean = acts + 6 * PF;
  float *dZ3 = work, *tA = dZ3 + PF, *tB = tA + PF, *dY3 = tB + PF, *uA = dY3 + PF, *uB = uA + PF;
  const float* P = params;
  float* G = grads;
  HeadBwdArgs h{};
  h.h3 = H3; h.g3 = G3; h.mean = mean; h.mw = P + L->mw;
  h.logstd = P + L->logstd; h.vw3 = P + L->vw3; h.action = action; h.idx = idx; h.d_logprobs = d_logprobs;
  h.d_entropy = d_entropy; h.d_values = d_values; h.dz3 = dZ3; h.dy3 = dY3;
  h.g_mw = G + L->mw; h.g_mb = G + L->mb; h.g_logstd = G + L->logstd; h.g_vw3 = G + L->vw3;
  h.g_b2 = G + L->bb2; h.g_vb2 = G + L->vb2;
  h.n = n; h.act = L->act_dim; h.vdim = L->value_dim;
  float* amax = work + 6 * PF;
  {
    cudaError_t ce = cudaMemsetAsync(amax, 0, 8 * sizeof(float), st);
    if (ce != cudaSuccess) return (int)ce;
  }
  h.amax_dz3 = amax;
  h.amax_dy3 = amax + 3;
  const int acc_len = (L->act_dim + L->value_dim) * kH + 64 + 2 * kH, w_len = (L->act_dim + L->value_dim) * kH;
  int nw = (232448 / 4 - w_len) / acc_len;
  nw = nw > 8 ? 8 : nw;
  const size_t smem = sizeof(float) * ((size_t)w_len + (size_t)nw * acc_len);
  const bool reg = L->act_dim <= 8 && L->value_dim <= 2;
  const int grid = head_grid(n);
  if (!(h.part = rb::partials_scratch((int64_t)grid * acc_len))) return RB200_E_UNSUPPORTED;
  {
    cudaError_t ce = cudaFuncSetAttribute(head_bwd_kernel<false>, cudaFuncAttributeMaxDynamicSharedMemorySize, (int)smem);
    if (ce == cudaSuccess)
      ce = cudaFuncSetAttribute(head_bwd_kernel<true>, cudaFuncAttributeMaxDynamicSharedMemorySize, (int)smem);
    if (ce != cudaSuccess) return (int)ce;
  }
  if (reg)
    head_bwd_kernel<true><<<grid, 32 * nw, smem, st>>>(h);
  else
    head_bwd_kernel<false><<<grid, 32 * nw, smem, st>>>(h);
  rb::count_launch();
  {
    cudaError_t ce = cudaPeekAtLastError();
    if (ce != cudaSuccess) return (int)ce;
  }
  {
    rb::tch::SlotSums ss{};
    ss.nslab = grid;
    ss.stride = acc_len;
    const int A = L->act_dim, V = L->value_dim;
    auto seg = [&](int off, float* out, int len) {
      ss.part[ss.count] = h.part + off; ss.out[ss.count] = out; ss.len[ss.count++] = len;
    };
    seg(0, h.g_mw, A * kH);
    seg((A + V) * kH, h.g_mb, A);
    seg((A + V) * kH + 32, h.g_logstd, A);
    seg((A + V) * kH + 64, h.g_b2, kH);
    if (d_values) {
      seg(A * kH, h.g_vw3, V * kH);
      seg((A + V) * kH + 64 + kH, h.g_vb2, kH);
    }
    if ((e = rb::tch::sum_slots(ss, st))) return e;
  }
  float* act_buf = const_cast<float*>(acts);
  TowerIO t[2] = {tower_io(L, P, wsplit, false, act_buf, n), tower_io(L, P, wsplit, true, act_buf + 3 * PF, n)};
  t[0].dZ3 = dZ3; t[0].tA = tA; t[0].tB = tB; t[0].amax = amax;
  t[0].g_w0 = G + L->bw0; t[0].g_b0 = G + L->bb0; t[0].g_w1 = G + L->bw1; t[0].g_b1 = G + L->bb1;
  t[0].g_w2 = G + L->bw2; t[0].g_b2 = G + L->bb2;
  t[1].dZ3 = dY3; t[1].tA = uA; t[1].tB = uB; t[1].amax = amax + 3;
  t[1].g_w0 = G + L->vw0; t[1].g_b0 = G + L->vb0; t[1].g_w1 = G + L->vw1; t[1].g_b1 = G + L->vb1;
  t[1].g_w2 = G + L->vw2; t[1].g_b2 = G + L->vb2;
  return towers_backward_h(states, idx, n, L->obs_dim, t, d_values ? 2 : 1, x_amax_slot(L, act_buf, n), st);
}

extern "C" int rb200_mlp_sample(const rb200_mlp_layout* L, const float* params, const float* wsplit,
                                const float* states, const float* noise, uint64_t seed, uint64_t offset,
                                const uint64_t* counter_dev, int64_t n, float* action, float* logprobs, float* values,
                                float* work, rb200_stream_t stream) {
  int e = check_layout(L);
  if (e) return e;
  if (!params || !wsplit || !states || !action || !logprobs || !work) return RB200_E_NULL;
  if (n <= 0) return RB200_E_SHAPE;
  cudaStream_t st = rb::as_stream(stream);
  if ((e = forward_towers(L, params, wsplit, states, nullptr, n, true, values != nullptr, work, nullptr, st))) return e;
  HeadFwdArgs h{};
  h.noise = noise; h.seed = seed; h.offset = offset; h.counter = counter_dev; h.sample_mode = 1; h.action_out = action;
  h.logprobs = logprobs;
  return head_forward(L, params, work, n, values, h, st);
}

namespace rb {
int mlp_mean_forward(const rb200_mlp_layout* L, const float* params, const float* wsplit, const float* states,
                     int64_t n, float* action, float* logprobs, float* values, float* work, cudaStream_t st) {
  int e = check_layout(L);
  if (e) return e;
  if ((e = forward_towers(L, params, wsplit, states, nullptr, n, true, values != nullptr, work, nullptr, st))) return e;
  HeadFwdArgs h{};
  h.sample_mode = 2; h.action_out = action; h.logprobs = logprobs;
  return head_forward(L, params, work, n, values, h, st);
}
}

extern "C" int rb200_absmax(const float* x, int64_t rows, int cols, float* out, rb200_stream_t stream) {
  if (!x || !out) return RB200_E_NULL;
  if (rows <= 0 || cols <= 0 || cols % 4 != 0) return RB200_E_SHAPE;
  return publish_absmax(x, rows, cols, out, rb::as_stream(stream));
}

namespace {
__global__ void __launch_bounds__(256) value_head_kernel(const float* __restrict__ g3, const float* __restrict__ vw3, float* __restrict__ values,
                                                         int64_t n, int vdim) {
  const int lane = threadIdx.x & 31, warp = threadIdx.x >> 5, nwarp = blockDim.x >> 5;
  for (int64_t row = (int64_t)blockIdx.x * nwarp + warp; row < n; row += (int64_t)gridDim.x * nwarp) {
    const float4 g0 = *reinterpret_cast<const float4*>(g3 + row * kH + lane * 4);
    const float4 g1 = *reinterpret_cast<const float4*>(g3 + row * kH + 128 + lane * 4);
    for (int c = 0; c < vdim; ++c) {
      const float4 w0 = *reinterpret_cast<const float4*>(vw3 + c * kH + lane * 4);
      const float4 w1 = *reinterpret_cast<const float4*>(vw3 + c * kH + 128 + lane * 4);
      float s = g0.x * w0.x + g0.y * w0.y + g0.z * w0.z + g0.w * w0.w + g1.x * w1.x + g1.y * w1.y + g1.z * w1.z +
                g1.w * w1.w;
      s = rb::warp_sum(s);
      if (lane == 0) values[row * vdim + c] = s;
    }
  }
}
}

extern "C" int rb200_mlp_value(const rb200_mlp_layout* L, const float* params, const float* wsplit,
                               const float* states, int64_t n, float* values, float* work, rb200_stream_t stream) {
  int e = check_layout(L);
  if (e) return e;
  if (!params || !wsplit || !states || !values || !work) return RB200_E_NULL;
  if (n <= 0 || L->value_dim <= 0) return RB200_E_SHAPE;
  cudaStream_t st = rb::as_stream(stream);
  if ((e = forward_towers(L, params, wsplit, states, nullptr, n, false, true, work, nullptr, st))) return e;
  value_head_kernel<<<head_grid(n), 256, 0, st>>>(work + 5 * act_floats(n), params + L->vw3, values, n, L->value_dim);
  rb::count_launch();
  RB_RETURN_LAUNCH();
}
```

### rlinf_b200/ops.py

```python
from __future__ import annotations

import ctypes as C
from typing import Optional

import torch

from . import _lib as L


def loss_mask(dones: torch.Tensor):
    lib = L.load()
    if dones.dim() != 3:
        raise ValueError(f"dones must be [n_chunk_steps+1, bsz, num_action_chunks], got {tuple(dones.shape)}")
    d = L.as_u8(L.to_device(dones))
    ncp1, B, Cc = d.shape
    mask = torch.empty((ncp1 - 1, B, Cc), dtype=torch.uint8, device=d.device)
    msum = torch.empty((B,), dtype=torch.int64, device=d.device)
    L.check(lib.rb200_loss_mask(L.ptr(d), L.ptr(mask), L.ptr(msum), ncp1 - 1, B, Cc, L.stream_ptr()), "loss_mask")
    return mask.view(torch.bool), msum.view(1, B, 1).expand(ncp1 - 1, B, Cc)


def gae(rewards, values, dones, gamma, gae_lambda, loss_mask=None, want_stats=False):
    lib = L.load()
    r = L.to_device(rewards, dtype=torch.float32)
    dev = r.device
    v = L.to_device(values, dev, torch.float32)
    d = L.as_u8(L.to_device(dones, dev))
    m = L.as_u8(L.to_device(loss_mask, dev))
    T, B = r.shape
    if d.shape != (T + 1, B):
        raise ValueError(f"dones must be [T+1,B]=({T + 1},{B}), got {tuple(d.shape)}")
    if v is not None and v.shape != (T + 1, B):
        raise ValueError(f"values must be [T+1,B]=({T + 1},{B}), got {tuple(v.shape)}")
    if m is not None and m.shape != (T, B):
        raise ValueError(f"loss_mask must be [T,B]=({T},{B}), got {tuple(m.shape)}")
    adv = torch.empty_like(r)
    ret = torch.empty_like(r)
    stats = torch.empty(6, dtype=torch.float64, device=dev) if want_stats else None
    L.check(lib.rb200_gae(L.ptr(r), L.ptr(v), L.ptr(d), L.ptr(m), L.ptr(adv), L.ptr(ret), L.ptr(stats), T, B,
                          float(gamma), float(gae_lambda), L.stream_ptr()), "gae")
    return adv, ret, stats


def normalize_(x: torch.Tensor, stats: torch.Tensor, eps: float = 1e-5) -> torch.Tensor:
    lib = L.load()
    L.check(lib.rb200_normalize(L.ptr(x), L.ptr(stats), x.numel(), float(eps), L.stream_ptr()), "normalize")
    return x


def grpo_scores(rewards, dones) -> torch.Tensor:
    lib = L.load()
    r = L.to_device(rewards, dtype=torch.float32)
    d = L.as_u8(L.to_device(dones, r.device))
    T, B = r.shape
    s = torch.empty((B,), dtype=torch.float32, device=r.device)
    L.check(lib.rb200_grpo_scores(L.ptr(r), L.ptr(d), L.ptr(s), T, B, L.stream_ptr()), "grpo_scores")
    return s


def grpo_advantages(scores, loss_mask, T, group_size, eps=1e-6) -> torch.Tensor:
    lib = L.load()
    s = L.to_device(scores, dtype=torch.float32).reshape(-1)
    m = L.as_u8(L.to_device(loss_mask, s.device))
    B = s.numel()
    adv = torch.empty((T, B), dtype=torch.float32, device=s.device)
    L.check(lib.rb200_grpo_advantages(L.ptr(s), L.ptr(m), L.ptr(adv), T, B, int(group_size), float(eps),
                                      L.stream_ptr()), "grpo_advantages")
    return adv


def absmax(x: torch.Tensor, out: Optional[torch.Tensor] = None) -> torch.Tensor:
    lib = L.load()
    rows, cols = x.shape[0], x[0].numel()
    out = out if out is not None else torch.empty(4 + cols if cols <= 256 else 1, dtype=torch.float32, device=x.device)
    L.check(lib.rb200_absmax(L.ptr(x), rows, cols, L.ptr(out), L.stream_ptr()), "absmax")
    return out


def gather_rows(src: torch.Tensor, idx: torch.Tensor) -> torch.Tensor:
    lib = L.load()
    s = L.to_device(src)
    i = L.to_device(idx, s.device, torch.int64)
    n_src = s.shape[0]
    row_bytes = s[0].numel() * s.element_size() if n_src > 0 else 0
    out = torch.empty((i.numel(), *s.shape[1:]), dtype=s.dtype, device=s.device)
    if i.numel() == 0 or row_bytes == 0:
        return out
    L.check(lib.rb200_gather_rows(L.ptr(s), L.ptr(i), L.ptr(out), i.numel(), n_src, row_bytes, L.stream_ptr()),
            "gather_rows")
    return out


def ppo_loss(*, logprobs, old_logprobs, advantages, C_chunks, A_dim, logprob_type, values=None, returns=None,
             prev_values=None, loss_mask=None, loss_mask_sum=None, mask_sum_row_mod=0, idx=None, entropy=None,
             adv_stats=None, adv_norm_eps=1e-5, clip_ratio_low=0.2, clip_ratio_high=0.2, clip_ratio_c=None,
             clip_log_ratio_min=None, clip_log_ratio_max=None, value_clip=0.0, huber_delta=0.0,
             max_episode_steps=None, critic_warmup=False, entropy_bonus=0.0, loss_scale=1.0, want_grads=True,
             _decoupled=None):
    lib = L.load()
    dev = logprobs.device
    bsz = logprobs.shape[0]
    with_critic = values is not None
    lp = logprobs.contiguous()
    a = L.PpoArgs()
    a.bsz, a.C, a.A = bsz, int(C_chunks), int(A_dim)
    a.logprob_type = L.LOGPROB_TYPES[logprob_type] if isinstance(logprob_type, str) else int(logprob_type)
    a.with_critic = 1 if with_critic else 0
    keep = [lp]

    def P(t, dtype=None):
        if t is None:
            return None
        t = L.to_device(t, dev, dtype)
        keep.append(t)
        return L.ptr(t)

    a.logprobs = L.ptr(lp)
    a.values = P(values, torch.float32)
    a.entropy = P(entropy, torch.float32)
    a.idx = P(idx, torch.int64)
    a.old_logprobs = P(old_logprobs, torch.float32)
    a.advantages = P(advantages, torch.float32)
    a.returns = P(returns, torch.float32)
    a.prev_values = P(prev_values, torch.float32)
    a.loss_mask = P(L.as_u8(loss_mask) if loss_mask is not None else None)
    a.loss_mask_sum = P(loss_mask_sum, torch.int64)
    a.mask_sum_row_mod = int(mask_sum_row_mod)
    a.adv_stats = P(adv_stats, torch.float64)
    a.adv_norm_eps = float(adv_norm_eps)
    a.clip_ratio_low, a.clip_ratio_high = float(clip_ratio_low), float(clip_ratio_high)
    a.clip_ratio_c = float(clip_ratio_c) if clip_ratio_c is not None else 0.0
    if clip_ratio_c is not None and not clip_ratio_c > 1.0:
        raise AssertionError("clip_ratio_c must be greater than 1.0")
    a.has_clip_log_ratio_min = int(clip_log_ratio_min is not None)
    a.has_clip_log_ratio_max = int(clip_log_ratio_max is not None)
    a.clip_log_ratio_min = float(clip_log_ratio_min or 0.0)
    a.clip_log_ratio_max = float(clip_log_ratio_max or 0.0)
    a.value_clip = float(value_clip or 0.0)
    a.huber_delta = float(huber_delta or 0.0)
    a.max_episode_steps = int(max_episode_steps) if max_episode_steps else 0
    a.critic_warmup = int(bool(critic_warmup))
    a.entropy_bonus = float(entropy_bonus)
    a.loss_scale = float(loss_scale)
    ws = _loss_workspace(dev)
    loss = torch.empty(1, dtype=torch.float32, device=dev)
    metrics = torch.empty(L.NUM_METRICS, dtype=torch.float32, device=dev)
    d_lp = torch.empty_like(lp) if want_grads else None
    d_v = torch.empty((values.numel(),), dtype=torch.float32, device=dev).view(values.shape) if (want_grads and with_critic) else None
    d_e = torch.empty_like(keep[0]) if (want_grads and entropy is not None) else None
    a.workspace, a.loss, a.metrics = L.ptr(ws), L.ptr(loss), L.ptr(metrics)
    a.d_logprobs, a.d_values, a.d_entropy = L.ptr(d_lp), L.ptr(d_v), L.ptr(d_e)
    if _decoupled is not None and _decoupled.get("version") is not None:
        if _decoupled.get("versions") is not None or _decoupled.get("current_version") is None:
            raise ValueError("a scalar `version` needs `current_version` and excludes the `versions` tensor")
        d = L.DppoScalarVersionArgs()
        d.base = a
        d.proximal_logprobs = P(_decoupled.get("proximal_logprobs"), torch.float32)
        d.version, d.current_version = float(_decoupled["version"]), float(_decoupled["current_version"])
        thr = _decoupled.get("behave_weight_threshold")
        d.has_behave_weight_threshold, d.behave_weight_threshold = int(thr is not None), float(thr or 0.0)
        L.check(lib.rb200_decoupled_ppo_loss_scalar_version(C.byref(d), L.stream_ptr()), "decoupled_ppo_loss")
        return loss, metrics, d_lp, d_v, d_e
    if _decoupled is not None:
        d = L.DppoArgs()
        d.base = a
        d.proximal_logprobs = P(_decoupled.get("proximal_logprobs"), torch.float32)
        d.versions = P(_decoupled.get("versions"), torch.float32)
        cv, thr = _decoupled.get("current_version"), _decoupled.get("behave_weight_threshold")
        d.has_current_version, d.current_version = int(cv is not None), float(cv or 0.0)
        d.has_behave_weight_threshold, d.behave_weight_threshold = int(thr is not None), float(thr or 0.0)
        L.check(lib.rb200_decoupled_ppo_loss(C.byref(d), L.stream_ptr()), "decoupled_ppo_loss")
        return loss, metrics, d_lp, d_v, d_e
    L.check(lib.rb200_ppo_loss(C.byref(a), L.stream_ptr()), "ppo_loss")
    return loss, metrics, d_lp, d_v, d_e


def opd_loss(*, logprobs, advantages, loss_mask, loss_mask_sum, max_episode_steps=None, loss_scale=1.0, want_grads=True):
    lib = L.load()
    lp = logprobs.contiguous()
    dev = lp.device
    n_units, g = lp.shape
    adv = L.to_device(advantages, dev, torch.float32).reshape(n_units, g)
    m = L.as_u8(L.to_device(loss_mask, dev)).reshape(n_units).contiguous()
    ms = L.to_device(loss_mask_sum, dev, torch.int64).reshape(n_units).contiguous()
    loss = torch.empty(1, dtype=torch.float32, device=dev)
    metrics = torch.empty(L.NUM_METRICS, dtype=torch.float32, device=dev)
    d_lp = torch.empty_like(lp) if want_grads else None
    L.check(lib.rb200_opd_loss(L.ptr(lp), L.ptr(adv), L.ptr(m), L.ptr(ms), n_units, g, int(max_episode_steps or 0),
                               float(loss_scale), L.ptr(_loss_workspace(dev)), L.ptr(loss), L.ptr(metrics), L.ptr(d_lp),
                               L.stream_ptr()), "opd_loss")
    return loss, metrics, d_lp


_WS: dict = {}


def _loss_workspace(dev) -> torch.Tensor:
    key = dev.index
    ws = _WS.get(key)
    if ws is None:
        ws = torch.zeros(32, dtype=torch.float64, device=dev)
        _WS[key] = ws
    return ws


def scale_(x: torch.Tensor, s: float) -> torch.Tensor:
    lib = L.load()
    L.check(lib.rb200_scale(L.ptr(x), x.numel(), float(s), L.stream_ptr()), "scale")
    return x


def scale_by_(x: torch.Tensor, s_dev: torch.Tensor) -> torch.Tensor:
    lib = L.load()
    s = s_dev.reshape(1).to(torch.float32)
    L.check(lib.rb200_scale_by(L.ptr(x), x.numel(), L.ptr(s), L.stream_ptr()), "scale_by")
    return x


def reward_filter(rewards, loss_mask, group_size, lower, upper):
    lib = L.load()
    r = L.to_device(rewards, dtype=torch.float32)
    m = L.as_u8(L.to_device(loss_mask, r.device))
    nc, B, Cc = r.shape
    if B % group_size != 0:
        raise AssertionError(f"batch {B} not divisible by group_size {group_size}")
    out = torch.empty((nc, B, Cc if m is not None else 1), dtype=torch.uint8, device=r.device)
    keep = torch.empty((B,), dtype=torch.uint8, device=r.device)
    L.check(lib.rb200_reward_filter(L.ptr(r), L.ptr(m), L.ptr(out), L.ptr(keep), nc, B, Cc, int(group_size),
                                    float(lower), float(upper), L.stream_ptr()), "reward_filter")
    return out.view(torch.bool)


_KL_MODES = {"kl": 0, "k1": 0, "abs": 1, "mse": 2, "k2": 2, "low_var_kl": 3, "k3": 3}


def kl_penalty_raw(logprob, ref_logprob, kind, want_grad=False):
    lib = L.load()
    if kind not in _KL_MODES:
        raise NotImplementedError(kind)
    a = L.to_device(logprob, dtype=torch.float32)
    b = L.to_device(ref_logprob, a.device, torch.float32)
    out = torch.empty_like(a)
    g = torch.empty_like(a) if want_grad else None
    L.check(lib.rb200_kl_penalty(L.ptr(a), L.ptr(b), L.ptr(out), L.ptr(g), a.numel(), _KL_MODES[kind],
                                 L.stream_ptr()), "kl_penalty")
    return out, g


_KL_ORDERS = {"megatron": 0, "fsdp": 1}


def _rows(t, name, shape, dev, dtype=torch.float32):
    if t is None:
        return None, 0
    if tuple(t.shape) != shape:
        raise ValueError(f"token_policy_loss: {name} has shape {tuple(t.shape)}, expected {shape} (that of logprobs)")
    if t.dtype != dtype:
        raise ValueError(f"token_policy_loss: {name} must be {dtype}, got {t.dtype}")
    if t.device != dev:
        raise ValueError(f"token_policy_loss: {name} is on {t.device}, logprobs on {dev}")
    if t.stride(1) != 1 or t.stride(0) < shape[1]:
        t = t.contiguous()
    return t, t.stride(0)


def _token_loss_cfg(logprobs, old_logprobs, advantages, loss_mask, entropy, ref_logprobs, rollout_logprobs,
                    recomputed_logprobs, loss_agg, clip_ratio_low, clip_ratio_high, clip_ratio_c, clip_log_ratio_min,
                    clip_log_ratio_max, entropy_bonus, kl_beta, kl_penalty, kl_order, importance_sampling_fix,
                    importance_sampling_clip, fast_path_zero_loss_mask):
    for name, t in (("logprobs", logprobs), ("old_logprobs", old_logprobs), ("advantages", advantages)):
        assert t.dtype == torch.float32, f"{name} must be float32 to keep numerical stability"
    if logprobs.dim() != 2:
        raise ValueError(f"token_policy_loss: logprobs must be [bsz, L], got {tuple(logprobs.shape)}")
    if loss_agg not in L.AGG_MODES:
        raise ValueError(f"Unsupported loss aggregation method: {loss_agg}; supported: {sorted(L.AGG_MODES)}")
    if clip_ratio_c is not None:
        assert clip_ratio_c > 1.0, "clip_ratio_c must be greater than 1.0"
    if kl_penalty == "full":
        raise NotImplementedError("kl_penalty 'full' needs the whole vocabulary's log-probs (utils.py:60-62)")
    if kl_penalty not in _KL_MODES:
        raise ValueError(f"unknown kl_penalty {kl_penalty!r}; supported: {sorted(_KL_MODES)}")
    if kl_order not in _KL_ORDERS:
        raise ValueError(f"kl_order must be one of {sorted(_KL_ORDERS)}, got {kl_order!r}")
    if importance_sampling_fix:
        if rollout_logprobs is None or recomputed_logprobs is None:
            raise ValueError("importance_sampling_fix requires both rollout_logprobs and recomputed_logprobs")
        if importance_sampling_clip is None:
            raise ValueError("importance_sampling_fix requires importance_sampling_clip")
    shape, dev = tuple(logprobs.shape), logprobs.device
    if loss_mask is None or tuple(loss_mask.shape) != shape:
        raise ValueError(f"token_policy_loss: loss_mask has shape {None if loss_mask is None else tuple(loss_mask.shape)}"
                         f", expected {shape} (that of logprobs)")
    if loss_mask.dtype not in (torch.bool, torch.uint8):
        raise ValueError(f"token_policy_loss: loss_mask must be bool or uint8, got {loss_mask.dtype}")
    if 0 in shape:
        raise ValueError(f"token_policy_loss: empty logprobs {shape}")
    named = dict(logprobs=logprobs, old_logprobs=old_logprobs, advantages=advantages,
                 loss_mask=loss_mask.view(torch.uint8) if loss_mask.dtype == torch.bool else loss_mask,
                 entropy=entropy, ref_logprobs=ref_logprobs, rollout_logprobs=rollout_logprobs,
                 recomputed_logprobs=recomputed_logprobs)
    ins = {k: _rows(t, k, shape, dev, torch.uint8 if k == "loss_mask" else torch.float32) for k, t in named.items()}
    hp = dict(clip_ratio_low=float(clip_ratio_low), clip_ratio_high=float(clip_ratio_high),
              clip_ratio_c=float(clip_ratio_c) if clip_ratio_c is not None else 0.0,
              has_clip_log_ratio_min=int(clip_log_ratio_min is not None),
              has_clip_log_ratio_max=int(clip_log_ratio_max is not None),
              clip_log_ratio_min=float(clip_log_ratio_min or 0.0), clip_log_ratio_max=float(clip_log_ratio_max or 0.0),
              entropy_bonus=float(entropy_bonus or 0.0), kl_beta=float(kl_beta or 0.0),
              importance_sampling_clip=float(importance_sampling_clip or 0.0), agg=L.AGG_MODES[loss_agg],
              kl_mode=_KL_MODES[kl_penalty], kl_order=_KL_ORDERS[kl_order],
              importance_sampling_fix=int(bool(importance_sampling_fix)),
              fast_path_zero_loss_mask=int(bool(fast_path_zero_loss_mask)))
    return ins, hp


def _token_loss_launch(lp, ent, ins, hp, want_d_lp, want_d_ent):
    if not lp.is_cuda:
        raise L.Rb200Error("token_policy_loss takes CUDA tensors; there is no CPU path")
    lib = L.load()
    dev = lp.device
    bsz, Ln = lp.shape
    a = L.TokenLossArgs()
    a.bsz, a.L = bsz, Ln
    keep = []
    for name, (t, stride) in ins.items():
        if name == "logprobs":
            t, stride = lp, lp.stride(0)
        elif name == "entropy":
            t, stride = ent, (ent.stride(0) if ent is not None else 0)
        keep.append(t)
        setattr(a, name, None if t is None else C.c_void_p(t.data_ptr()))
        setattr(a, name + "_stride", stride)
    for k, v in hp.items():
        setattr(a, k, v)
    wsb = L.load().rb200_token_loss_workspace_bytes(bsz, Ln)
    if wsb < 0:
        raise ValueError(f"token_policy_loss: unsupported shape bsz={bsz} L={Ln} (bsz <= 65535)")
    ws = torch.empty(wsb, dtype=torch.uint8, device=dev)
    loss = torch.empty(1, dtype=torch.float32, device=dev)
    metrics = torch.empty(L.TM_NUM, dtype=torch.float32, device=dev)
    d_lp = torch.empty((bsz, Ln), dtype=torch.float32, device=dev) if want_d_lp else None
    d_ent = torch.empty((bsz, Ln), dtype=torch.float32, device=dev) if want_d_ent else None
    a.workspace, a.workspace_bytes = L.ptr(ws), wsb
    a.loss, a.metrics, a.d_logprobs, a.d_entropy = L.ptr(loss), L.ptr(metrics), L.ptr(d_lp), L.ptr(d_ent)
    L.check(lib.rb200_token_ppo_loss(C.byref(a), L.stream_ptr(dev)), "token_ppo_loss")
    return loss.reshape(()), metrics, d_lp, d_ent


class _TokenPolicyLoss(torch.autograd.Function):

    @staticmethod
    def forward(ctx, logprobs, entropy, ins, hp):
        want_d_ent = entropy is not None and ctx.needs_input_grad[1] and hp["entropy_bonus"] > 0.0
        loss, metrics, d_lp, d_ent = _token_loss_launch(logprobs.detach(), None if entropy is None else entropy.detach(),
                                                        ins, hp, ctx.needs_input_grad[0], want_d_ent)
        ctx.grads = (d_lp, d_ent)
        ctx.mark_non_differentiable(metrics)
        return loss, metrics

    @staticmethod
    def backward(ctx, g_loss, _g_metrics):
        d_lp, d_ent = ctx.grads
        ctx.grads = None
        if d_lp is not None:
            scale_by_(d_lp, g_loss)
        if d_ent is not None:
            scale_by_(d_ent, g_loss)
        return d_lp, d_ent, None, None


def token_policy_loss(logprobs, old_logprobs, advantages, loss_mask, *, entropy=None, ref_logprobs=None,
                      rollout_logprobs=None, recomputed_logprobs=None, loss_agg: str = "token-mean",
                      clip_ratio_low: float = 0.2, clip_ratio_high: float = 0.2, clip_ratio_c: Optional[float] = None,
                      clip_log_ratio_min: Optional[float] = None, clip_log_ratio_max: Optional[float] = None,
                      entropy_bonus: float = 0.0, kl_beta: float = 0.0, kl_penalty: str = "kl", kl_order: str = "fsdp",
                      importance_sampling_fix: bool = False, importance_sampling_clip: Optional[float] = None,
                      fast_path_zero_loss_mask: bool = False):
    ins, hp = _token_loss_cfg(logprobs, old_logprobs, advantages, loss_mask, entropy, ref_logprobs, rollout_logprobs,
                              recomputed_logprobs, loss_agg, clip_ratio_low, clip_ratio_high, clip_ratio_c,
                              clip_log_ratio_min, clip_log_ratio_max, entropy_bonus, kl_beta, kl_penalty, kl_order,
                              importance_sampling_fix, importance_sampling_clip, fast_path_zero_loss_mask)
    lp, _ = ins["logprobs"]
    ent, _ = ins["entropy"]
    needs = torch.is_grad_enabled() and (logprobs.requires_grad or (entropy is not None and entropy.requires_grad))
    if needs:
        loss, metrics = _TokenPolicyLoss.apply(lp, ent, ins, hp)
    else:
        loss, metrics, _, _ = _token_loss_launch(lp, ent, ins, hp, False, False)
    with_rr = rollout_logprobs is not None and recomputed_logprobs is not None
    keys = {s: k for s, k in L.TM_KEYS.items() if k != "actor/rollout_train_kl" or with_rr}
    return loss, {k: metrics[s] for s, k in keys.items()}


def masked_stats(x, mask=None, mask_div=1):
    lib = L.load()
    xs = L.to_device(x, dtype=torch.float32).contiguous()
    m = L.as_u8(L.to_device(mask, xs.device))
    out = torch.empty(4, dtype=torch.float64, device=xs.device)
    L.check(lib.rb200_masked_stats(L.ptr(xs), L.ptr(m.contiguous() if m is not None else None), xs.numel(),
                                   int(mask_div), L.ptr(out), L.stream_ptr()), "masked_stats")
    return out


def masked_moments(x, mask=None) -> torch.Tensor:
    lib = L.load()
    xs = L.to_device(x, dtype=torch.float32).contiguous()
    m = L.as_u8(L.to_device(mask, xs.device))
    if m is not None:
        if m.shape != xs.shape:
            raise AssertionError((tuple(m.shape), tuple(xs.shape)))
        m = m.contiguous()
    out = torch.empty(3, dtype=torch.float64, device=xs.device)
    L.check(lib.rb200_masked_moments(L.ptr(xs), L.ptr(m), xs.numel(), L.ptr(out), L.stream_ptr()), "masked_moments")
    return out


def masked_normalize(x, stats3, mask=None, mode=0, eps=1e-5, unbiased=False) -> torch.Tensor:
    lib = L.load()
    xs = L.to_device(x, dtype=torch.float32).contiguous()
    m = L.as_u8(L.to_device(mask, xs.device))
    m = m.contiguous() if m is not None else None
    out = torch.empty_like(xs)
    st = L.to_device(stats3, xs.device, torch.float64)
    L.check(lib.rb200_masked_normalize(L.ptr(xs), L.ptr(m), L.ptr(out), xs.numel(), L.ptr(st), int(mode), float(eps),
                                       int(bool(unbiased)), L.stream_ptr()), "masked_normalize")
    return out


def raw_advantages(scores, loss_mask, want_stats=False):
    lib = L.load()
    s = L.to_device(scores, dtype=torch.float32).reshape(-1).contiguous()
    m = L.as_u8(L.to_device(loss_mask, s.device)).contiguous()
    Ln, B = m.shape
    if s.numel() != B:
        raise RuntimeError(f"{s.numel()} scores for a loss_mask of {tuple(m.shape)}")
    adv = torch.empty((Ln, B), dtype=torch.float32, device=s.device)
    stats = torch.empty(3, dtype=torch.float64, device=s.device) if want_stats else None
    L.check(lib.rb200_raw_advantages(L.ptr(s), L.ptr(m), L.ptr(adv), Ln, B, L.ptr(stats), L.stream_ptr()), "raw_advantages")
    return adv, stats


def reinpp_returns(rewards, loss_mask, kl_beta=0.0, logprob=None, ref_logprob=None, kl_kind="k1"):
    lib = L.load()
    r = L.to_device(rewards, dtype=torch.float32).reshape(-1).contiguous()
    m = L.as_u8(L.to_device(loss_mask, r.device)).contiguous()
    Ln, B = m.shape
    if r.numel() != B:
        raise RuntimeError(f"{r.numel()} rewards for a loss_mask of {tuple(m.shape)}")
    lp = rlp = None
    if kl_beta > 0:
        if kl_kind not in _KL_MODES:
            raise NotImplementedError(kl_kind)
        lp = L.to_device(logprob, r.device, torch.float32).contiguous()
        rlp = L.to_device(ref_logprob, r.device, torch.float32).contiguous()
        if lp.shape != m.shape or rlp.shape != m.shape:
# ... 917 lines not shown
```

### rlinf_b200/policy.py

```python
from __future__ import annotations

import ctypes as C
import math
from typing import Optional

import torch

from . import _lib as L

HIDDEN = 256


class MLPPolicy:
    def __init__(self, obs_dim: int, action_dim: int, num_action_chunks: int = 1, add_value_head: bool = True,
                 value_granularity: str = "action_level", device=None, seed: Optional[int] = None):
        self.obs_dim, self.action_dim, self.num_action_chunks = int(obs_dim), int(action_dim), int(num_action_chunks)
        self.act_dim = self.action_dim * self.num_action_chunks
        self.value_dim = 0 if not add_value_head else (1 if value_granularity == "chunk_level" else self.num_action_chunks)
        self.device = device or L.default_device()
        lib = L.load()
        self.layout = L.MlpLayout()
        L.check(lib.rb200_mlp_layout_init(C.byref(self.layout), self.obs_dim, self.act_dim, self.value_dim, HIDDEN),
                "mlp_layout_init")
        n = self.layout.total
        self._param_store = torch.zeros(n + 4, dtype=torch.float32, device=self.device)
        self.flat_params = self._param_store[:n]
        self.flat_grads = torch.zeros(n, dtype=torch.float32, device=self.device)
        self._spec = self._build_spec()
        self._scratch: dict[tuple, torch.Tensor] = {}
        self.wsplit = torch.zeros(int(lib.rb200_mlp_wsplit_floats(C.byref(self.layout))), dtype=torch.float32,
                                  device=self.device)
        self._wsplit_fresh = False
        self.reset_parameters(seed)

    def _build_spec(self):
        Lo, H, O, A, V = self.layout, HIDDEN, self.obs_dim, self.act_dim, self.value_dim
        spec = [("actor_logstd", Lo.logstd, (1, A)),
                ("value_head.mlp.0.weight", Lo.vw0, (H, O)), ("value_head.mlp.0.bias", Lo.vb0, (H,)),
                ("value_head.mlp.2.weight", Lo.vw1, (H, H)), ("value_head.mlp.2.bias", Lo.vb1, (H,)),
                ("value_head.mlp.4.weight", Lo.vw2, (H, H)), ("value_head.mlp.4.bias", Lo.vb2, (H,)),
                ("value_head.mlp.6.weight", Lo.vw3, (V, H)),
                ("backbone.0.weight", Lo.bw0, (H, O)), ("backbone.0.bias", Lo.bb0, (H,)),
                ("backbone.2.weight", Lo.bw1, (H, H)), ("backbone.2.bias", Lo.bb1, (H,)),
                ("backbone.4.weight", Lo.bw2, (H, H)), ("backbone.4.bias", Lo.bb2, (H,)),
                ("actor_mean.weight", Lo.mw, (A, H)), ("actor_mean.bias", Lo.mb, (A,))]
        if V == 0:
            spec = [s for s in spec if not s[0].startswith("value_head")]
        return spec

    def named_parameters(self):
        for name, off, shape in self._spec:
            yield name, self.flat_params[off: off + math.prod(shape)].view(shape)

    def named_grads(self):
        for name, off, shape in self._spec:
            yield name, self.flat_grads[off: off + math.prod(shape)].view(shape)

    def state_dict(self):
        return {k: v.clone() for k, v in self.named_parameters()}

    def sync_buffer(self) -> torch.Tensor:
        return self._param_store[: self.flat_params.numel() + 1]

    def mark_params_changed(self):
        self._wsplit_fresh = False

    def _ws(self):
        if not self._wsplit_fresh:
            L.check(L.load().rb200_mlp_prepare_weights(C.byref(self.layout), L.ptr(self.flat_params),
                                                       L.ptr(self.wsplit), L.stream_ptr()), "mlp_prepare_weights")
            self._wsplit_fresh = True
        return L.ptr(self.wsplit)

    def load_state_dict(self, sd: dict, strict: bool = False):
        views = dict(self.named_parameters())
        if strict:
            unexpected = [k for k in sd if k not in views]
            shapes = [f"{k}: {tuple(sd[k].shape)} vs {tuple(v.shape)}" for k, v in views.items()
                      if k in sd and tuple(sd[k].shape) != tuple(v.shape)]
            if unexpected or shapes:
                raise ValueError(f"state dict does not match the policy: unexpected keys {unexpected}, "
                                 f"shape mismatches {shapes}")
        missing = [k for k in views if k not in sd]
        if missing:
            raise KeyError(f"missing parameters: {missing}")
        for k, v in views.items():
            v.copy_(sd[k].to(self.device, torch.float32).reshape(v.shape))
        self.mark_params_changed()

    def lr_group_ends(self):
        segs = []
        for name, off, shape in self._spec:
            kind = "critic" if "value_head" in name else "actor"
            end = off + math.prod(shape)
            if segs and segs[-1][0] == kind:
                segs[-1][1] = end
            else:
                segs.append([kind, end])
        segs[-1][1] = int(self.layout.total)
        return segs

    def reset_parameters(self, seed: Optional[int] = None):
        g = torch.Generator().manual_seed(0 if seed is None else int(seed))
        for name, p in self.named_parameters():
            if name == "actor_logstd":
                p.fill_(-0.5)
            elif name.endswith("bias"):
                p.zero_()
            elif name == "value_head.mlp.6.weight":
                p.copy_(torch.randn(p.shape, generator=g) * 0.02)
            elif name.startswith("value_head"):
                p.copy_(torch.randn(p.shape, generator=g) * ((5.0 / 3.0) / math.sqrt(p.shape[0])))
            else:
                w = torch.empty(p.shape)
                gain = 0.01 * math.sqrt(2) if name.startswith("actor_mean") else math.sqrt(2)
                torch.nn.init.orthogonal_(w, gain=gain, generator=g)
                p.copy_(w)
        self.mark_params_changed()

    def _buf(self, key, numel):
        t = self._scratch.get(key)
        if t is None or t.numel() < numel:
            t = torch.empty(numel, dtype=torch.float32, device=self.device)
            self._scratch[key] = t
        return t

    def forward_train(self, states, action, idx=None, n=None, compute_entropy=True, compute_values=True,
                      states_amax=None):
        lib = L.load()
        n = int(n if n is not None else (idx.numel() if idx is not None else states.shape[0]))
        nscr = lib.rb200_mlp_fwd_scratch_floats(C.byref(self.layout), n)
        acts = self._buf("acts", nscr)
        work = self._buf("work", nscr)
        logp = torch.empty((n, self.act_dim), dtype=torch.float32, device=self.device)
        ent = torch.empty_like(logp) if compute_entropy else None
        vals = torch.empty((n, self.value_dim), dtype=torch.float32, device=self.device) if (
            compute_values and self.value_dim > 0) else None
        L.check(lib.rb200_mlp_forward(C.byref(self.layout), L.ptr(self.flat_params), self._ws(), L.ptr(states),
                                      L.ptr(action), L.ptr(idx), n, L.ptr(logp), L.ptr(ent), L.ptr(vals), L.ptr(acts),
                                      L.ptr(work), L.ptr(states_amax), L.stream_ptr()), "mlp_forward")
        self._last = (states, action, idx, n, acts)
        out = {"logprobs": logp}
        if ent is not None:
            out["entropy"] = ent
        if vals is not None:
            out["values"] = vals
        return out

    def backward(self, d_logprobs, d_values=None, d_entropy=None):
        lib = L.load()
        states, action, idx, n, acts = self._last
        work = self._buf("work", acts.numel())
        L.check(lib.rb200_mlp_backward(C.byref(self.layout), L.ptr(self.flat_params), self._ws(), L.ptr(states),
                                       L.ptr(action), L.ptr(idx), n, L.ptr(d_logprobs), L.ptr(d_entropy), L.ptr(d_values),
                                       L.ptr(acts), L.ptr(work), L.ptr(self.flat_grads), L.stream_ptr()),
                "mlp_backward")

    def sample(self, states, noise=None, seed=0, offset=0, calculate_values=True, counter=None, out=None):
        lib = L.load()
        n = states.shape[0]
        work = self._buf("sample", lib.rb200_mlp_fwd_scratch_floats(C.byref(self.layout), n))
        if out is not None:
            action, logp, vals = out
        else:
            action = torch.empty((n, self.act_dim), dtype=torch.float32, device=self.device)
            logp = torch.empty_like(action)
            vals = torch.empty((n, self.value_dim), dtype=torch.float32, device=self.device) if (
                calculate_values and self.value_dim > 0) else None
        L.check(lib.rb200_mlp_sample(C.byref(self.layout), L.ptr(self.flat_params), self._ws(), L.ptr(states), L.ptr(noise),
                                     int(seed), int(offset), L.ptr(counter), n, L.ptr(action), L.ptr(logp),
                                     L.ptr(vals), L.ptr(work), L.stream_ptr()), "mlp_sample")
        return action, logp, vals

    def value(self, states, out=None):
        lib = L.load()
        n = states.shape[0]
        work = self._buf("value", lib.rb200_mlp_fwd_scratch_floats(C.byref(self.layout), n))
        vals = out if out is not None else torch.empty((n, self.value_dim), dtype=torch.float32, device=self.device)
        L.check(lib.rb200_mlp_value(C.byref(self.layout), L.ptr(self.flat_params), self._ws(), L.ptr(states), n, L.ptr(vals),
                                    L.ptr(work), L.stream_ptr()), "mlp_value")
        return vals

    def mean(self, states, calculate_logprobs=True, calculate_values=True, out=None, work_key="mean"):
        lib = L.load()
        n = states.shape[0]
        work = self._buf(work_key, lib.rb200_mlp_fwd_scratch_floats(C.byref(self.layout), n))
        action = out if out is not None else torch.empty((n, self.act_dim), dtype=torch.float32, device=self.device)
        logp = torch.empty_like(action) if calculate_logprobs else None
        vals = torch.empty((n, self.value_dim), dtype=torch.float32, device=self.device) if (
            calculate_values and self.value_dim > 0) else None
        L.check(lib.rb200_mlp_mean(C.byref(self.layout), L.ptr(self.flat_params), self._ws(), L.ptr(states), n,
                                   L.ptr(action), L.ptr(logp), L.ptr(vals), L.ptr(work), L.stream_ptr()), "mlp_mean")
        return action, logp, vals

    def predict_action_batch(self, env_obs, calculate_values=True, noise=None, seed=0, offset=0, mode="train",
                             **kwargs):
        states = env_obs["states"]
        if mode == "train":
            action, logp, vals = self.sample(states, noise=noise, seed=seed, offset=offset,
                                             calculate_values=calculate_values)
        elif mode == "eval":
            action, logp, vals = self.mean(states, calculate_values=calculate_values)
        else:
            raise NotImplementedError(f"mode={mode!r}")
        if vals is None:
            vals = torch.zeros((states.shape[0], 1), dtype=torch.float32, device=self.device)
        result = {"prev_logprobs": logp, "prev_values": vals,
                  "forward_inputs": {"action": action, "model_action": action, "states": states}}
        return action.reshape(-1, self.num_action_chunks, self.action_dim), result


class FlatAdamW:

    def __init__(self, policy: MLPPolicy, lr=3e-4, value_lr=3e-4, betas=(0.9, 0.999), eps=1e-8, weight_decay=1e-2,
                 clip_grad=0.5):
        self.policy = policy
        self.lr, self.value_lr, self.betas, self.eps, self.weight_decay = lr, value_lr, betas, eps, weight_decay
        self.clip_grad = float(clip_grad)
        n = policy.flat_params.numel()
        dev = policy.device
        self.exp_avg = torch.zeros(n, dtype=torch.float32, device=dev)
        self.exp_avg_sq = torch.zeros(n, dtype=torch.float32, device=dev)
        self.grad_sq = torch.zeros(1, dtype=torch.float64, device=dev)
        self.state = torch.zeros(4, dtype=torch.float64, device=dev)
        segs = policy.lr_group_ends()
        self._ends = (C.c_int64 * len(segs))(*[e for _, e in segs])
        self._kinds = [k for k, _ in segs]
        self.lr_scale = 1.0
        self.frozen: set = set()
        self._lr_dev = torch.zeros(8, dtype=torch.float64, device=dev)
        self._lr_key = None

    def zero_grad(self):
        self.policy.flat_grads.zero_()

    def _segment_lrs(self):
        return [-1.0 if k in self.frozen else (self.value_lr if k == "critic" else self.lr) * self.lr_scale
                for k in self._kinds]

    def sync_lr_table(self):
        lrs = self._segment_lrs()
        key = tuple(lrs)
        if key != self._lr_key:
            host = torch.zeros(8, dtype=torch.float64)
            host[: len(lrs)] = torch.tensor(lrs, dtype=torch.float64)
            self._lr_dev.copy_(host)
            self._lr_key = key

    def step(self, grad_scale: float = 1.0):
        lib = L.load()
        p = self.policy
        n = p.flat_params.numel()
        st = L.stream_ptr()
        if not torch.cuda.is_current_stream_capturing():
            self.sync_lr_table()
        L.check(lib.rb200_grad_sqnorm(L.ptr(p.flat_grads), n, L.ptr(self.grad_sq), st), "grad_sqnorm")
        L.check(lib.rb200_adamw_step_dev(L.ptr(p.flat_params), L.ptr(p.flat_grads), L.ptr(self.exp_avg),
                                         L.ptr(self.exp_avg_sq), n, self._ends, L.ptr(self._lr_dev), len(self._kinds),
                                         self.betas[0], self.betas[1], self.eps, self.weight_decay, self.clip_grad,
                                         float(grad_scale), L.ptr(self.grad_sq), L.ptr(self.state), st), "adamw_step")
        self._last_grad_scale = float(grad_scale)
        p.mark_params_changed()

    def state_dict(self) -> dict:
        return {"exp_avg": self.exp_avg, "exp_avg_sq": self.exp_avg_sq, "state": self.state,
                "last_grad_scale": float(getattr(self, "_last_grad_scale", 1.0))}

    def load_state_dict(self, sd: dict):
        self.exp_avg.copy_(sd["exp_avg"])
        self.exp_avg_sq.copy_(sd["exp_avg_sq"])
        self.state.copy_(sd["state"])
        self._last_grad_scale = float(sd["last_grad_scale"])

    def reset_state(self, carry_grads: bool = False):
        self.state[0].zero_()
        if not carry_grads:
            self.exp_avg.zero_()
            self.exp_avg_sq.zero_()
            return
        gmul = self.state[2].to(torch.float32) * getattr(self, "_last_grad_scale", 1.0)
        g = self.policy.flat_grads * gmul
        g = torch.where(self.state[3] != 0, torch.zeros_like(g), g)
        torch.mul(g, 1.0 - self.betas[0], out=self.exp_avg)
        torch.mul(g * g, 1.0 - self.betas[1], out=self.exp_avg_sq)

    def last_grad_norm(self) -> torch.Tensor:
        return self.state[1]

    def lr_list(self):
        lrs = []
        if "actor" not in self.frozen:
            lrs.append(self.lr * self.lr_scale)
        if "critic" in self._kinds and "critic" not in self.frozen:
            lrs.append(self.value_lr * self.lr_scale)
        return lrs
```

Baseline: 6.608 million.

## Fuse policy head, PPO loss gradient and head backward into one kernel

Adds a training path that runs only the MLP towers forward, then a single kernel that computes head outputs, per-element PPO/value loss gradients and head weight gradients before handing off to the tower backward. This replaces the separate head forward, PPO loss kernel, and head backward launches, and avoids writing and re-reading logprob/value/gradient tensors. The actor falls back to the old path when the fused variant is unsupported. The catch is more complex kernels with heavy shared memory, a duplicate loss computation still launched for metrics, and extra Python setup per micro-batch.

```diff
diff --git a/include/rlinf_b200.h b/include/rlinf_b200.h
--- a/include/rlinf_b200.h
+++ b/include/rlinf_b200.h
@@ -273,6 +273,15 @@
                        const float* d_logprobs, const float* d_entropy, const float* d_values,
                        const float* acts, float* work, float* grads, rb200_stream_t stream);
 
+int rb200_mlp_forward_towers(const rb200_mlp_layout* L, const float* params, const float* wsplit,
+                             const float* states, const int64_t* idx, int64_t n, int with_values, float* acts,
+                             const float* states_amax, rb200_stream_t stream);
+int rb200_mlp_head_loss_supported(const rb200_mlp_layout* L, const rb200_ppo_args* ppo);
+int rb200_mlp_head_loss_backward(const rb200_mlp_layout* L, const float* params, const float* wsplit,
+                                 const float* states, const float* action, const int64_t* idx, int64_t n,
+                                 const rb200_ppo_args* ppo, const float* acts, float* work, float* grads,
+                                 rb200_stream_t stream);
+
 int rb200_mlp_sample(const rb200_mlp_layout* L, const float* params, const float* wsplit,
                      const float* states, const float* noise, uint64_t seed, uint64_t offset,
                      const uint64_t* counter_dev, int64_t n, float* action, float* logprobs, float* values,
diff --git a/rlinf_b200/_lib.py b/rlinf_b200/_lib.py
--- a/rlinf_b200/_lib.py
+++ b/rlinf_b200/_lib.py
@@ -170,6 +170,11 @@
     "rb200_mlp_forward": (c_int, [C.POINTER(MlpLayout)] + [c_void_p] * 5 + [c_int64] + [c_void_p] * 7),
     "rb200_absmax": (c_int, [c_void_p, c_int64, c_int, c_void_p, c_void_p]),
     "rb200_mlp_backward": (c_int, [C.POINTER(MlpLayout)] + [c_void_p] * 5 + [c_int64] + [c_void_p] * 7),
+    "rb200_mlp_forward_towers": (c_int, [C.POINTER(MlpLayout)] + [c_void_p] * 4 + [c_int64, c_int, c_void_p, c_void_p,
+                                                                                  c_void_p]),
+    "rb200_mlp_head_loss_supported": (c_int, [C.POINTER(MlpLayout), C.POINTER(PpoArgs)]),
+    "rb200_mlp_head_loss_backward": (c_int, [C.POINTER(MlpLayout)] + [c_void_p] * 5 + [c_int64, C.POINTER(PpoArgs)] +
+                                     [c_void_p] * 4),
     "rb200_mlp_sample": (c_int, [C.POINTER(MlpLayout)] + [c_void_p] * 4 + [c_uint64, c_uint64, c_void_p, c_int64] + [c_void_p] * 5),
     "rb200_tc_gemm_h": (c_int, [c_void_p, c_void_p, c_void_p, c_int64, c_int, c_int, c_void_p, c_void_p, c_void_p]),
     "rb200_tc_wgrad_h": (c_int, [c_void_p, c_void_p, c_void_p, c_int64, c_int, c_void_p, c_void_p]),
diff --git a/rlinf_b200/actor.py b/rlinf_b200/actor.py
--- a/rlinf_b200/actor.py
+++ b/rlinf_b200/actor.py
@@ -269,10 +269,8 @@
         with_critic = self._with_critic
         ent_bonus = float(cfg.algorithm.get("entropy_bonus", 0) or 0)
         warm = self.optimizer_steps < self.critic_warmup_steps
-        out = self.model.forward_train(fi["states"][lo:hi], fi["action"][lo:hi], compute_entropy=ent_bonus > 0,
-                                       compute_values=with_critic, states_amax=self._states_amax)
         A = cfg.actor.model.get("action_dim", 7)
-        Cc = out["logprobs"].shape[1] // A
+        Cc = self.model.act_dim // A
         U = 1 if cfg.algorithm.logprob_type == "chunk_level" else Cc
         n = hi - lo
 
@@ -280,9 +278,8 @@
             t = batch.get(key)
             return None if t is None else t[lo:hi].reshape(n, U)
 
-        loss, metrics, d_lp, d_v, d_e = ops.ppo_loss(
-            logprobs=out["logprobs"], values=out.get("values") if with_critic else None,
-            entropy=out.get("entropy"), old_logprobs=batch["prev_logprobs"][lo:hi].reshape(n, Cc * A),
+        ppo = dict(
+            old_logprobs=batch["prev_logprobs"][lo:hi].reshape(n, Cc * A),
             advantages=unit("advantages"), returns=unit("returns") if with_critic else None,
             prev_values=unit("prev_values") if with_critic else None, loss_mask=unit("loss_mask"),
             loss_mask_sum=unit("loss_mask_sum"), C_chunks=Cc, A_dim=A, logprob_type=cfg.algorithm.logprob_type,
@@ -290,6 +287,16 @@
             value_clip=cfg.algorithm.get("value_clip", None), huber_delta=cfg.algorithm.get("huber_delta", None),
             max_episode_steps=cfg.env.train.max_episode_steps if batch.get("loss_mask_sum") is not None else None,
             critic_warmup=warm, entropy_bonus=ent_bonus, loss_scale=1.0 / self.gradient_accumulation)
+        fused = self.model.forward_loss_backward(fi["states"][lo:hi], fi["action"][lo:hi], compute_entropy=ent_bonus > 0,
+                                                 compute_values=with_critic, states_amax=self._states_amax, **ppo)
+        if fused is not None:
+            metric_out.copy_(fused[1])
+            return
+        out = self.model.forward_train(fi["states"][lo:hi], fi["action"][lo:hi], compute_entropy=ent_bonus > 0,
+                                       compute_values=with_critic, states_amax=self._states_amax)
+        loss, metrics, d_lp, d_v, d_e = ops.ppo_loss(
+            logprobs=out["logprobs"], values=out.get("values") if with_critic else None, entropy=out.get("entropy"),
+            **ppo)
         metric_out.copy_(metrics)
         self.model.backward(d_lp, d_v if with_critic else None, d_e)
 
diff --git a/rlinf_b200/csrc/head_row.cuh b/rlinf_b200/csrc/head_row.cuh
--- /dev/null
+++ b/rlinf_b200/csrc/head_row.cuh
@@ -0,0 +1,34 @@
+#pragma once
+#include <cuda_runtime.h>
+
+namespace rb {
+namespace head {
+
+constexpr float kHalfLog2Pi = 0.91893853320467274178f;
+
+__device__ __forceinline__ float dot8(const float4& h0, const float4& h1, const float4& w0, const float4& w1) {
+  return h0.x * w0.x + h0.y * w0.y + h0.z * w0.z + h0.w * w0.w + h1.x * w1.x + h1.y * w1.y + h1.z * w1.z + h1.w * w1.w;
+}
+
+__device__ __forceinline__ float normal_logprob(float x, float mean, float sd) {
+  const float d = x - mean;
+  const float var = sd * sd;
+  return -(d * d) / (2.0f * var) - logf(sd) - kHalfLog2Pi;
+}
+
+__device__ __forceinline__ float normal_entropy(float sd) { return 0.5f + kHalfLog2Pi + logf(sd); }
+
+__device__ __forceinline__ float4 tanh_grad(const float4& dh, const float4& h) {
+  float4 o;
+  o.x = dh.x * (1.f - h.x * h.x); o.y = dh.y * (1.f - h.y * h.y);
+  o.z = dh.z * (1.f - h.z * h.z); o.w = dh.w * (1.f - h.w * h.w);
+  return o;
+}
+
+__device__ __forceinline__ float absmax4(const float4& a, const float4& b) {
+  return fmaxf(fmaxf(fmaxf(fabsf(a.x), fabsf(a.y)), fmaxf(fabsf(a.z), fabsf(a.w))),
+               fmaxf(fmaxf(fabsf(b.x), fabsf(b.y)), fmaxf(fabsf(b.z), fabsf(b.w))));
+}
+
+}
+}
diff --git a/rlinf_b200/csrc/mlp.cu b/rlinf_b200/csrc/mlp.cu
--- a/rlinf_b200/csrc/mlp.cu
+++ b/rlinf_b200/csrc/mlp.cu
@@ -1,6 +1,9 @@
 #include <curand_kernel.h>
 
 #include "common.cuh"
+#include "critic_unit.cuh"
+#include "head_row.cuh"
+#include "ppo_unit.cuh"
 #include "sgemm.cuh"
 #include "tc_gemm.cuh"
 
@@ -35,7 +38,6 @@
 constexpr int kH = 256;
 constexpr int kMaxAct = 32;
 constexpr int kMaxVal = 8;
-constexpr float kHalfLog2Pi = 0.91893853320467274178f;
 
 struct HeadFwdArgs {
   const float* h3;
@@ -89,9 +91,7 @@
     for (int a = 0; a < p.act; ++a) {
       const float4 w0 = *reinterpret_cast<const float4*>(s_mw + a * kH + lane * 4);
       const float4 w1 = *reinterpret_cast<const float4*>(s_mw + a * kH + 128 + lane * 4);
-      float s = h0.x * w0.x + h0.y * w0.y + h0.z * w0.z + h0.w * w0.w + h1.x * w1.x + h1.y * w1.y + h1.z * w1.z +
-                h1.w * w1.w;
-      s = rb::warp_sum(s);
+      const float s = rb::warp_sum(rb::head::dot8(h0, h1, w0, w1));
       if (lane == a) my_mean = s + p.mb[a];
     }
     if (lane < p.act) {
@@ -116,10 +116,8 @@
         const int64_t src = p.idx ? p.idx[row] : row;
         x = p.action[src * p.act + lane];
       }
-      const float d = x - my_mean;
-      const float var = sd * sd;
-      if (p.logprobs) p.logprobs[row * p.act + lane] = -(d * d) / (2.0f * var) - logf(sd) - kHalfLog2Pi;
-      if (p.entropy) p.entropy[row * p.act + lane] = 0.5f + kHalfLog2Pi + logf(sd);
+      if (p.logprobs) p.logprobs[row * p.act + lane] = rb::head::normal_logprob(x, my_mean, sd);
+      if (p.entropy) p.entropy[row * p.act + lane] = rb::head::normal_entropy(sd);
       if (p.mean_out) p.mean_out[row * p.act + lane] = my_mean;
     }
     if (want_v) {
@@ -127,9 +125,7 @@
       for (int c = 0; c < p.vdim; ++c) {
         const float4 w0 = *reinterpret_cast<const float4*>(s_vw + c * kH + lane * 4);
         const float4 w1 = *reinterpret_cast<const float4*>(s_vw + c * kH + 128 + lane * 4);
-        float s = g0.x * w0.x + g0.y * w0.y + g0.z * w0.z + g0.w * w0.w + g1.x * w1.x + g1.y * w1.y + g1.z * w1.z +
-                  g1.w * w1.w;
-        s = rb::warp_sum(s);
+        const float s = rb::warp_sum(rb::head::dot8(g0, g1, w0, w1));
         if (lane == 0) p.values[row * p.vdim + c] = s;
       }
     }
@@ -261,17 +257,12 @@
       atomicAdd(&am[128 + lane * 4 + 0], g * h1.x); atomicAdd(&am[128 + lane * 4 + 1], g * h1.y);
       atomicAdd(&am[128 + lane * 4 + 2], g * h1.z); atomicAdd(&am[128 + lane * 4 + 3], g * h1.w);
     }
-    float4 o0, o1;
-    o0.x = dh0.x * (1.f - h0.x * h0.x); o0.y = dh0.y * (1.f - h0.y * h0.y);
-    o0.z = dh0.z * (1.f - h0.z * h0.z); o0.w = dh0.w * (1.f - h0.w * h0.w);
-    o1.x = dh1.x * (1.f - h1.x * h1.x); o1.y = dh1.y * (1.f - h1.y * h1.y);
-    o1.z = dh1.z * (1.f - h1.z * h1.z); o1.w = dh1.w * (1.f - h1.w * h1.w);
+    const float4 o0 = rb::head::tanh_grad(dh0, h0), o1 = rb::head::tanh_grad(dh1, h1);
     *reinterpret_cast<float4*>(p.dz3 + row * kH + lane * 4) = o0;
     *reinterpret_cast<float4*>(p.dz3 + row * kH + 128 + lane * 4) = o1;
     cb[0] += o0.x; cb[1] += o0.y; cb[2] += o0.z; cb[3] += o0.w;
     cb[4] += o1.x; cb[5] += o1.y; cb[6] += o1.z; cb[7] += o1.w;
-    mz = fmaxf(mz, fmaxf(fmaxf(fmaxf(fabsf(o0.x), fabsf(o0.y)), fmaxf(fabsf(o0.z), fabsf(o0.w))),
-                         fmaxf(fmaxf(fabsf(o1.x), fabsf(o1.y)), fmaxf(fabsf(o1.z), fabsf(o1.w)))));
+    mz = fmaxf(mz, rb::head::absmax4(o0, o1));
 
     if (has_v) {
       const float4 g0 = cur.g0, g1 = cur.g1;
@@ -296,17 +287,12 @@
         atomicAdd(&av[128 + lane * 4 + 0], g * g1.x); atomicAdd(&av[128 + lane * 4 + 1], g * g1.y);
         atomicAdd(&av[128 + lane * 4 + 2], g * g1.z); atomicAdd(&av[128 + lane * 4 + 3], g * g1.w);
       }
-      float4 q0, q1;
-      q0.x = dg0.x * (1.f - g0.x * g0.x); q0.y = dg0.y * (1.f - g0.y * g0.y);
-      q0.z = dg0.z * (1.f - g0.z * g0.z); q0.w = dg0.w * (1.f - g0.w * g0.w);
-      q1.x = dg1.x * (1.f - g1.x * g1.x); q1.y = dg1.y * (1.f - g1.y * g1.y);
-      q1.z = dg1.z * (1.f - g1.z * g1.z); q1.w = dg1.w * (1.f - g1.w * g1.w);
+      const float4 q0 = rb::head::tanh_grad(dg0, g0), q1 = rb::head::tanh_grad(dg1, g1);
       *reinterpret_cast<float4*>(p.dy3 + row * kH + lane * 4) = q0;
       *reinterpret_cast<float4*>(p.dy3 + row * kH + 128 + lane * 4) = q1;
       cv[0] += q0.x; cv[1] += q0.y; cv[2] += q0.z; cv[3] += q0.w;
       cv[4] += q1.x; cv[5] += q1.y; cv[6] += q1.z; cv[7] += q1.w;
-      my = fmaxf(my, fmaxf(fmaxf(fmaxf(fabsf(q0.x), fabsf(q0.y)), fmaxf(fabsf(q0.z), fabsf(q0.w))),
-                           fmaxf(fmaxf(fabsf(q1.x), fabsf(q1.y)), fmaxf(fabsf(q1.z), fabsf(q1.w)))));
+      my = fmaxf(my, rb::head::absmax4(q0, q1));
     }
   }
   if (p.amax_dz3 != nullptr) {
@@ -351,6 +337,252 @@
           atomicAdd(&av[128 + lane * 4 + j], rv[c][4 + j]);
         }
       }
+    }
+  }
+  __syncthreads();
+  for (int i = threadIdx.x; i < acc_len; i += blockDim.x) {
+    float s = 0.f;
+    for (int w = 0; w < nwarp; ++w) s += acc0[w * acc_len + i];
+    p.part[(size_t)blockIdx.x * acc_len + i] = s;
+  }
+}
+
+struct LossHyper {
+  float clip_lo_bound, clip_hi_bound, dual_c;
+  int has_lr_min, has_lr_max;
+  float lr_min, lr_max;
+  float value_clip, huber_delta, half_huber_delta;
+  int critic_warmup;
+  float entropy_bonus, loss_scale, adv_eps;
+};
+
+struct HeadLossArgs {
+  const float *h3, *g3, *mw, *mb, *logstd, *vw3, *action;
+  const int64_t* idx;
+  const float* old_logprobs;
+  const float* advantages;
+  const float* returns;
+  const float* prev_values;
+  const double* adv_stats;
+  float* logprobs;
+  float* entropy;
+  float* values;
+  float *dz3, *dy3, *amax_dz3, *amax_dy3, *part;
+  int64_t n;
+  int act, vdim, U, g, with_critic;
+  LossHyper h;
+};
+
+__global__ void __launch_bounds__(256, 2) head_loss_bwd_kernel(HeadLossArgs p) {
+  extern __shared__ float sm[];
+  const int lane = threadIdx.x & 31, warp = threadIdx.x >> 5, nwarp = blockDim.x >> 5;
+  const int acc_len = (p.act + p.vdim) * kH + 64 + 2 * kH;
+  float* s_mw = sm;
+  float* s_vw = s_mw + p.act * kH;
+  float* acc0 = s_vw + p.vdim * kH;
+  float* a_mw = acc0 + warp * acc_len;
+  float* a_vw = a_mw + p.act * kH;
+  float* a_mb = a_vw + p.vdim * kH;
+  float* a_ls = a_mb + 32;
+  float* a_b2 = a_ls + 32;
+  float* a_vb2 = a_b2 + kH;
+  const bool has_v = p.with_critic != 0;
+  for (int i = threadIdx.x; i < p.act * kH; i += blockDim.x) s_mw[i] = p.mw[i];
+  for (int i = threadIdx.x; i < p.vdim * kH; i += blockDim.x) s_vw[i] = has_v ? p.vw3[i] : 0.f;
+  for (int i = threadIdx.x; i < nwarp * acc_len; i += blockDim.x) acc0[i] = 0.f;
+  __syncthreads();
+
+  const double n_units = (double)(p.n * p.U);
+  const float coef_actor = (float)(1.0 / n_units), coef_unit = (float)(1.0 / n_units);
+  bool norm_adv = false;
+  float adv_mean = 0.0f, adv_den = 1.0f;
+  if (p.adv_stats != nullptr && p.adv_stats[0] > 0.0) {
+    const double cnt = p.adv_stats[0];
+    const double mean_d = p.adv_stats[1] / cnt;
+    const double var_d = (p.adv_stats[2] - p.adv_stats[1] * mean_d) / (cnt - 1.0);
+    adv_mean = (float)mean_d;
+    adv_den = __fadd_rn((float)sqrt(var_d > 0.0 || !(var_d == var_d) ? var_d : 0.0), p.h.adv_eps);
+    norm_adv = true;
+  }
+  const float scale = p.h.loss_scale;
+  const float den = (p.entropy && p.h.entropy_bonus > 0.0f && !p.h.critic_warmup)
+                        ? -scale * p.h.entropy_bonus * (float)(1.0 / n_units) : 0.0f;
+
+  const bool act_lane = lane < p.act;
+  const int unit = act_lane ? lane / p.g : 0;
+  const float sd_l = act_lane ? expf(p.logstd[lane]) : 1.f;
+
+  float cb[8] = {0.f, 0.f, 0.f, 0.f, 0.f, 0.f, 0.f, 0.f}, cv[8] = {0.f, 0.f, 0.f, 0.f, 0.f, 0.f, 0.f, 0.f};
+  float mz = 0.f, my = 0.f;
+  struct RowIn {
+    float4 h0, h1, g0, g1;
+    float x, old;
+  };
+  auto load_row = [&](int64_t row) -> RowIn {
+    RowIn r;
+    r.h0 = r.h1 = r.g0 = r.g1 = make_float4(0.f, 0.f, 0.f, 0.f);
+    r.x = r.old = 0.f;
+    if (row < p.n) {
+      r.h0 = __ldg(reinterpret_cast<const float4*>(p.h3 + row * kH + lane * 4));
+      r.h1 = __ldg(reinterpret_cast<const float4*>(p.h3 + row * kH + 128 + lane * 4));
+      if (has_v) {
+        r.g0 = __ldg(reinterpret_cast<const float4*>(p.g3 + row * kH + lane * 4));
+        r.g1 = __ldg(reinterpret_cast<const float4*>(p.g3 + row * kH + 128 + lane * 4));
+      }
+      if (act_lane) {
+        const int64_t src = p.idx ? p.idx[row] : row;
+        r.x = __ldg(p.action + src * p.act + lane);
+        r.old = __ldg(p.old_logprobs + row * p.act + lane);
+      }
+    }
+    return r;
+  };
+  const int64_t row_stride = (int64_t)gridDim.x * nwarp;
+  const int64_t row_first = (int64_t)blockIdx.x * nwarp + warp;
+  RowIn nxt0 = load_row(row_first), nxt1 = load_row(row_first + row_stride);
+  for (int64_t row = row_first; row < p.n; row += row_stride) {
+    const RowIn cur = nxt0;
+    nxt0 = nxt1;
+    nxt1 = load_row(row + 2 * row_stride);
+    const float4 h0 = cur.h0, h1 = cur.h1;
+    float adv = act_lane ? __ldg(p.advantages + row * p.U + unit) : 0.f;
+    float rt0 = 0.f, pv0 = 0.f, rt1 = 0.f, pv1 = 0.f;
+    if (has_v) {
+      rt0 = __ldg(p.returns + row * p.U);
+      pv0 = __ldg(p.prev_values + row * p.U);
+      if (p.vdim > 1) {
+        rt1 = __ldg(p.returns + row * p.U + 1);
+        pv1 = __ldg(p.prev_values + row * p.U + 1);
+      }
+    }
+
+    float v[8];
+#pragma unroll
+    for (int a = 0; a < 8; ++a) {
+      v[a] = 0.f;
+      if (a < p.act) {
+        const float4 w0 = *reinterpret_cast<const float4*>(s_mw + a * kH + lane * 4);
+        const float4 w1 = *reinterpret_cast<const float4*>(s_mw + a * kH + 128 + lane * 4);
+        v[a] = rb::head::dot8(h0, h1, w0, w1);
+      }
+    }
+    const bool b4 = lane & 16, b3 = lane & 8, b2 = lane & 4;
+#pragma unroll
+    for (int j = 0; j < 4; ++j) {
+      const float send = b4 ? v[j] : v[4 + j];
+      v[j] = (b4 ? v[4 + j] : v[j]) + __shfl_xor_sync(0xffffffffu, send, 16);
+    }
+#pragma unroll
+    for (int j = 0; j < 2; ++j) {
+      const float send = b3 ? v[j] : v[2 + j];
+      v[j] = (b3 ? v[2 + j] : v[j]) + __shfl_xor_sync(0xffffffffu, send, 8);
+    }
+    {
+      const float send = b2 ? v[0] : v[1];
+      v[0] = (b2 ? v[1] : v[0]) + __shfl_xor_sync(0xffffffffu, send, 4);
+    }
+    v[0] += __shfl_xor_sync(0xffffffffu, v[0], 2);
+    v[0] += __shfl_xor_sync(0xffffffffu, v[0], 1);
+    const float mu = __shfl_sync(0xffffffffu, v[0], (lane & 7) * 4) + (act_lane ? __ldg(p.mb + lane) : 0.f);
+    const float lp = act_lane ? rb::head::normal_logprob(cur.x, mu, sd_l) : 0.f;
+    if (act_lane) {
+      p.logprobs[row * p.act + lane] = lp;
+      if (p.entropy) p.entropy[row * p.act + lane] = rb::head::normal_entropy(sd_l);
+    }
+
+    float lp_u = 0.0f, old_u = 0.0f;
+    for (int k = 0; k < p.g; ++k) {
+      lp_u = __fadd_rn(lp_u, __shfl_sync(0xffffffffu, lp, unit * p.g + k));
+      old_u = __fadd_rn(old_u, __shfl_sync(0xffffffffu, cur.old, unit * p.g + k));
+    }
+    if (norm_adv) adv = __fdiv_rn(__fsub_rn(adv, adv_mean), adv_den);
+    const rb::RatioOut o = rb::ratio_terms(lp_u, old_u, adv, true, p.h);
+    const float dlp = p.h.critic_warmup ? 0.0f : scale * coef_actor * o.dL_dlp;
+
+    float dmu = 0.f;
+    if (act_lane) {
+      const float var_l = sd_l * sd_l;
+      const float d = cur.x - mu;
+      dmu = dlp * d / var_l;
+      const float dls = dlp * (d * d / var_l - 1.0f) + den;
+      atomicAdd(&a_mb[lane], dmu);
+      atomicAdd(&a_ls[lane], dls);
+    }
+    float4 dh0 = make_float4(0.f, 0.f, 0.f, 0.f), dh1 = dh0;
+#pragma unroll
+    for (int a = 0; a < 8; ++a) {
+      if (a >= p.act) break;
+      const float g = __shfl_sync(0xffffffffu, dmu, a);
+      const float4 w0 = *reinterpret_cast<const float4*>(s_mw + a * kH + lane * 4);
+      const float4 w1 = *reinterpret_cast<const float4*>(s_mw + a * kH + 128 + lane * 4);
+      dh0.x += g * w0.x; dh0.y += g * w0.y; dh0.z += g * w0.z; dh0.w += g * w0.w;
+      dh1.x += g * w1.x; dh1.y += g * w1.y; dh1.z += g * w1.z; dh1.w += g * w1.w;
+      float4* am0 = reinterpret_cast<float4*>(a_mw + a * kH + lane * 4);
+      float4* am1 = reinterpret_cast<float4*>(a_mw + a * kH + 128 + lane * 4);
+      float4 m0 = *am0, m1 = *am1;
+      m0.x = __fmaf_rn(g, h0.x, m0.x); m0.y = __fmaf_rn(g, h0.y, m0.y); m0.z = __fmaf_rn(g, h0.z, m0.z);
+      m0.w = __fmaf_rn(g, h0.w, m0.w);
+      m1.x = __fmaf_rn(g, h1.x, m1.x); m1.y = __fmaf_rn(g, h1.y, m1.y); m1.z = __fmaf_rn(g, h1.z, m1.z);
+      m1.w = __fmaf_rn(g, h1.w, m1.w);
+      *am0 = m0;
+      *am1 = m1;
+    }
+    const float4 o0 = rb::head::tanh_grad(dh0, h0), o1 = rb::head::tanh_grad(dh1, h1);
+    *reinterpret_cast<float4*>(p.dz3 + row * kH + lane * 4) = o0;
+    *reinterpret_cast<float4*>(p.dz3 + row * kH + 128 + lane * 4) = o1;
+    cb[0] += o0.x; cb[1] += o0.y; cb[2] += o0.z; cb[3] += o0.w;
+    cb[4] += o1.x; cb[5] += o1.y; cb[6] += o1.z; cb[7] += o1.w;
+    mz = fmaxf(mz, rb::head::absmax4(o0, o1));
+
+    if (has_v) {
+      const float4 g0 = cur.g0, g1 = cur.g1;
+      float4 dg0 = make_float4(0.f, 0.f, 0.f, 0.f), dg1 = dg0;
+#pragma unroll
+      for (int c = 0; c < 2; ++c) {
+        if (c >= p.vdim) break;
+        const float4 w0 = *reinterpret_cast<const float4*>(s_vw + c * kH + lane * 4);
+        const float4 w1 = *reinterpret_cast<const float4*>(s_vw + c * kH + 128 + lane * 4);
+        const float v = rb::warp_sum(rb::head::dot8(g0, g1, w0, w1));
+        if (lane == 0) p.values[row * p.vdim + c] = v;
+        const rb::CriticOut co = rb::critic_terms(v, c == 0 ? pv0 : pv1, c == 0 ? rt0 : rt1,
+                                                  p.h.value_clip, p.h.huber_delta, p.h.half_huber_delta);
+        const float g = scale * coef_unit * rb::critic_dvl(co, p.h.value_clip, p.h.huber_delta);
+        dg0.x += g * w0.x; dg0.y += g * w0.y; dg0.z += g * w0.z; dg0.w += g * w0.w;
+        dg1.x += g * w1.x; dg1.y += g * w1.y; dg1.z += g * w1.z; dg1.w += g * w1.w;
+        float4* av0 = reinterpret_cast<float4*>(a_vw + c * kH + lane * 4);
+        float4* av1 = reinterpret_cast<float4*>(a_vw + c * kH + 128 + lane * 4);
+        float4 m0 = *av0, m1 = *av1;
+        m0.x = __fmaf_rn(g, g0.x, m0.x); m0.y = __fmaf_rn(g, g0.y, m0.y); m0.z = __fmaf_rn(g, g0.z, m0.z);
+        m0.w = __fmaf_rn(g, g0.w, m0.w);
+        m1.x = __fmaf_rn(g, g1.x, m1.x); m1.y = __fmaf_rn(g, g1.y, m1.y); m1.z = __fmaf_rn(g, g1.z, m1.z);
+        m1.w = __fmaf_rn(g, g1.w, m1.w);
+        *av0 = m0;
+        *av1 = m1;
+      }
+      const float4 q0 = rb::head::tanh_grad(dg0, g0), q1 = rb::head::tanh_grad(dg1, g1);
+      *reinterpret_cast<float4*>(p.dy3 + row * kH + lane * 4) = q0;
+      *reinterpret_cast<float4*>(p.dy3 + row * kH + 128 + lane * 4) = q1;
+      cv[0] += q0.x; cv[1] += q0.y; cv[2] += q0.z; cv[3] += q0.w;
+      cv[4] += q1.x; cv[5] += q1.y; cv[6] += q1.z; cv[7] += q1.w;
+      my = fmaxf(my, rb::head::absmax4(q0, q1));
+    }
+  }
+#pragma unroll
+  for (int o = 16; o > 0; o >>= 1) {
+    mz = fmaxf(mz, __shfl_xor_sync(0xffffffffu, mz, o));
+    my = fmaxf(my, __shfl_xor_sync(0xffffffffu, my, o));
+  }
+  if (lane == 0) {
+    if (mz > 0.f) atomicMax(reinterpret_cast<unsigned int*>(p.amax_dz3), __float_as_uint(mz));
+    if (has_v && my > 0.f) atomicMax(reinterpret_cast<unsigned int*>(p.amax_dy3), __float_as_uint(my));
+  }
+#pragma unroll
+  for (int j = 0; j < 4; ++j) {
+    atomicAdd(&a_b2[lane * 4 + j], cb[j]);
+    atomicAdd(&a_b2[128 + lane * 4 + j], cb[4 + j]);
+    if (has_v) {
+      atomicAdd(&a_vb2[lane * 4 + j], cv[j]);
+      atomicAdd(&a_vb2[128 + lane * 4 + j], cv[4 + j]);
     }
   }
   __syncthreads();
@@ -631,6 +863,58 @@
   return head_forward(L, params, acts, n, values, h, st);
 }
 
+namespace {
+struct HeadBwdLaunch {
+  int acc_len, nw;
+  size_t smem;
+};
+HeadBwdLaunch head_bwd_launch(const rb200_mlp_layout* L) {
+  HeadBwdLaunch c;
+  c.acc_len = (L->act_dim + L->value_dim) * kH + 64 + 2 * kH;
+  const int w_len = (L->act_dim + L->value_dim) * kH;
+  int nw = (232448 / 4 - w_len) / c.acc_len;
+  c.nw = nw > 8 ? 8 : nw;
+  c.smem = sizeof(float) * ((size_t)w_len + (size_t)c.nw * c.acc_len);
+  return c;
+}
+
+int head_grads_and_towers(const rb200_mlp_layout* L, const float* P, const float* wsplit, const float* states,
+                          const int64_t* idx, int64_t n, const float* part, int grid, bool with_v, const float* acts,
+                          float* work, float* G, cudaStream_t st) {
+  int e;
+  const int64_t PF = act_floats(n);
+  float *dZ3 = work, *tA = dZ3 + PF, *tB = tA + PF, *dY3 = tB + PF, *uA = dY3 + PF, *uB = uA + PF;
+  float* amax = work + 6 * PF;
+  {
+    rb::tch::SlotSums ss{};
+    ss.nslab = grid;
+    ss.stride = (L->act_dim + L->value_dim) * kH + 64 + 2 * kH;
+    const int A = L->act_dim, V = L->value_dim;
+    auto seg = [&](int off, float* out, int len) {
+      ss.part[ss.count] = part + off; ss.out[ss.count] = out; ss.len[ss.count++] = len;
+    };
+    seg(0, G + L->mw, A * kH);
+    seg((A + V) * kH, G + L->mb, A);
+    seg((A + V) * kH + 32, G + L->logstd, A);
+    seg((A + V) * kH + 64, G + L->bb2, kH);
+    if (with_v) {
+      seg(A * kH, G + L->vw3, V * kH);
+      seg((A + V) * kH + 64 + kH, G + L->vb2, kH);
+    }
+    if ((e = rb::tch::sum_slots(ss, st))) return e;
+  }
+  float* act_buf = const_cast<float*>(acts);
+  TowerIO t[2] = {tower_io(L, P, wsplit, false, act_buf, n), tower_io(L, P, wsplit, true, act_buf + 3 * PF, n)};
+  t[0].dZ3 = dZ3; t[0].tA = tA; t[0].tB = tB; t[0].amax = amax;
+  t[0].g_w0 = G + L->bw0; t[0].g_b0 = G + L->bb0; t[0].g_w1 = G + L->bw1; t[0].g_b1 = G + L->bb1;
+  t[0].g_w2 = G + L->bw2; t[0].g_b2 = G + L->bb2;
+  t[1].dZ3 = dY3; t[1].tA = uA; t[1].tB = uB; t[1].amax = amax + 3;
+  t[1].g_w0 = G + L->vw0; t[1].g_b0 = G + L->vb0; t[1].g_w1 = G + L->vw1; t[1].g_b1 = G + L->vb1;
+  t[1].g_w2 = G + L->vw2; t[1].g_b2 = G + L->vb2;
+  return towers_backward_h(states, idx, n, L->obs_dim, t, with_v ? 2 : 1, x_amax_slot(L, act_buf, n), st);
+}
+}
+
 extern "C" int rb200_mlp_backward(const rb200_mlp_layout* L, const float* params, const float* wsplit,
                                   const float* states, const float* action, const int64_t* idx, int64_t n,
                                   const float* d_logprobs, const float* d_entropy, const float* d_values,
@@ -642,7 +926,7 @@
   cudaStream_t st = rb::as_stream(stream);
   const int64_t PF = act_floats(n);
   const float *H3 = acts + 2 * PF, *G3 = acts + 5 * PF, *mean = acts + 6 * PF;
-  float *dZ3 = work, *tA = dZ3 + PF, *tB = tA + PF, *dY3 = tB + PF, *uA = dY3 + PF, *uB = uA + PF;
+  float *dZ3 = work, *dY3 = work + 3 * PF;
   const float* P = params;
   float* G = grads;
   HeadBwdArgs h{};
@@ -659,10 +943,9 @@
   }
   h.amax_dz3 = amax;
   h.amax_dy3 = amax + 3;
-  const int acc_len = (L->act_dim + L->value_dim) * kH + 64 + 2 * kH, w_len = (L->act_dim + L->value_dim) * kH;
-  int nw = (232448 / 4 - w_len) / acc_len;
-  nw = nw > 8 ? 8 : nw;
-  const size_t smem = sizeof(float) * ((size_t)w_len + (size_t)nw * acc_len);
+  const HeadBwdLaunch c = head_bwd_launch(L);
+  const int acc_len = c.acc_len, nw = c.nw;
+  const size_t smem = c.smem;
   const bool reg = L->act_dim <= 8 && L->value_dim <= 2;
   const int grid = head_grid(n);
   if (!(h.part = rb::partials_scratch((int64_t)grid * acc_len))) return RB200_E_UNSUPPORTED;
@@ -681,33 +964,97 @@
     cudaError_t ce = cudaPeekAtLastError();
     if (ce != cudaSuccess) return (int)ce;
   }
+  return head_grads_and_towers(L, P, wsplit, states, idx, n, h.part, grid, d_values != nullptr, acts, work, G, st);
+}
+
+extern "C" int rb200_mlp_forward_towers(const rb200_mlp_layout* L, const float* params, const float* wsplit,
+                                        const float* states, const int64_t* idx, int64_t n, int with_values,
+                                        float* acts, const float* states_amax, rb200_stream_t stream) {
+  int e = check_layout(L);
+  if (e) return e;
+  if (!params || !wsplit || !states || !acts) return RB200_E_NULL;
+  if (n <= 0) return RB200_E_SHAPE;
+  if (with_values && L->value_dim == 0) return RB200_E_SHAPE;
+  return forward_towers(L, params, wsplit, states, idx, n, true, with_values != 0, acts, states_amax,
+                        rb::as_stream(stream));
+}
+
+extern "C" int rb200_mlp_head_loss_supported(const rb200_mlp_layout* L, const rb200_ppo_args* a) {
+  if (check_layout(L) || !a) return 0;
+  const int U = a->logprob_type == RB200_LOGPROB_CHUNK ? 1 : a->C;
+  return L->act_dim <= 8 && L->value_dim <= 2 && a->logprob_type != RB200_LOGPROB_TOKEN && a->C * a->A == L->act_dim &&
+         !a->loss_mask && !a->idx && (!a->with_critic || L->value_dim == U) &&
+         !(a->entropy && a->logprob_type == RB200_LOGPROB_CHUNK && a->C != 1);
+}
+
+extern "C" int rb200_mlp_head_loss_backward(const rb200_mlp_layout* L, const float* params, const float* wsplit,
+                                            const float* states, const float* action, const int64_t* idx, int64_t n,
+                                            const rb200_ppo_args* ppo, const float* acts, float* work, float* grads,
+                                            rb200_stream_t stream) {
+  int e = check_layout(L);
+  if (e) return e;
+  if (!params || !wsplit || !states || !action || !ppo || !acts || !work || !grads) return RB200_E_NULL;
+  const rb200_ppo_args& a = *ppo;
+  if (n <= 0 || a.bsz != n) return RB200_E_SHAPE;
+  if (!a.logprobs || !a.old_logprobs || !a.advantages || !a.metrics || !a.workspace) return RB200_E_NULL;
+  if (a.with_critic && (!a.values || !a.returns || !a.prev_values)) return RB200_E_NULL;
+  if (a.d_logprobs || a.d_values || a.d_entropy) return RB200_E_ARG;
+  if (a.clip_ratio_c > 0.0 && !(a.clip_ratio_c > 1.0)) return RB200_E_ARG;
+  if (!rb200_mlp_head_loss_supported(L, ppo)) return RB200_E_UNSUPPORTED;
+  cudaStream_t st = rb::as_stream(stream);
+  const int64_t PF = act_floats(n);
+  const float* P = params;
+  HeadLossArgs h{};
+  h.h3 = acts + 2 * PF; h.g3 = acts + 5 * PF; h.mw = P + L->mw; h.mb = P + L->mb; h.logstd = P + L->logstd;
+  h.vw3 = P + L->vw3; h.action = action; h.idx = idx;
+  h.old_logprobs = a.old_logprobs; h.advantages = a.advantages; h.returns = a.returns; h.prev_values = a.prev_values;
+  h.adv_stats = a.adv_stats;
+  h.logprobs = const_cast<float*>(a.logprobs); h.entropy = const_cast<float*>(a.entropy);
+  h.values = const_cast<float*>(a.values);
+  h.dz3 = work; h.dy3 = work + 3 * PF;
+  h.n = n; h.act = L->act_dim; h.vdim = L->value_dim;
+  h.U = a.logprob_type == RB200_LOGPROB_CHUNK ? 1 : a.C;
+  h.g = L->act_dim / h.U;
+  h.with_critic = a.with_critic;
+  h.h.clip_lo_bound = (float)(1.0 - a.clip_ratio_low);
+  h.h.clip_hi_bound = (float)(1.0 + a.clip_ratio_high);
+  h.h.dual_c = a.clip_ratio_c > 0.0 ? (float)a.clip_ratio_c : 0.0f;
+  h.h.has_lr_min = a.has_clip_log_ratio_min;
+  h.h.has_lr_max = a.has_clip_log_ratio_max;
+  h.h.lr_min = (float)a.clip_log_ratio_min;
+  h.h.lr_max = (float)a.clip_log_ratio_max;
+  h.h.value_clip = (float)a.value_clip;
+  h.h.huber_delta = (float)a.huber_delta;
+  h.h.half_huber_delta = (float)(0.5 * a.huber_delta);
+  h.h.critic_warmup = a.critic_warmup;
+  h.h.entropy_bonus = (float)a.entropy_bonus;
+  h.h.loss_scale = (float)a.loss_scale;
+  h.h.adv_eps = a.adv_norm_eps;
+  float* amax = work + 6 * PF;
   {
-    rb::tch::SlotSums ss{};
-    ss.nslab = grid;
-    ss.stride = acc_len;
-    const int A = L->act_dim, V = L->value_dim;
-    auto seg = [&](int off, float* out, int len) {
-      ss.part[ss.count] = h.part + off; ss.out[ss.count] = out; ss.len[ss.count++] = len;
-    };
-    seg(0, h.g_mw, A * kH);
-    seg((A + V) * kH, h.g_mb, A);
-    seg((A + V) * kH + 32, h.g_logstd, A);
-    seg((A + V) * kH + 64, h.g_b2, kH);
-    if (d_values) {
-      seg(A * kH, h.g_vw3, V * kH);
-      seg((A + V) * kH + 64 + kH, h.g_vb2, kH);
-    }
-    if ((e = rb::tch::sum_slots(ss, st))) return e;
-  }
-  float* act_buf = const_cast<float*>(acts);
-  TowerIO t[2] = {tower_io(L, P, wsplit, false, act_buf, n), tower_io(L, P, wsplit, true, act_buf + 3 * PF, n)};
-  t[0].dZ3 = dZ3; t[0].tA = tA; t[0].tB = tB; t[0].amax = amax;
-  t[0].g_w0 = G + L->bw0; t[0].g_b0 = G + L->bb0; t[0].g_w1 = G + L->bw1; t[0].g_b1 = G + L->bb1;
-  t[0].g_w2 = G + L->bw2; t[0].g_b2 = G + L->bb2;
-  t[1].dZ3 = dY3; t[1].tA = uA; t[1].tB = uB; t[1].amax = amax + 3;
-  t[1].g_w0 = G + L->vw0; t[1].g_b0 = G + L->vb0; t[1].g_w1 = G + L->vw1; t[1].g_b1 = G + L->vb1;
-  t[1].g_w2 = G + L->vw2; t[1].g_b2 = G + L->vb2;
-  return towers_backward_h(states, idx, n, L->obs_dim, t, d_values ? 2 : 1, x_amax_slot(L, act_buf, n), st);
+    cudaError_t ce = cudaMemsetAsync(amax, 0, 8 * sizeof(float), st);
+    if (ce != cudaSuccess) return (int)ce;
+  }
+  h.amax_dz3 = amax;
+  h.amax_dy3 = amax + 3;
+  const HeadBwdLaunch c = head_bwd_launch(L);
+  const int grid = head_grid(n);
+  if (!(h.part = rb::partials_scratch((int64_t)grid * c.acc_len))) return RB200_E_UNSUPPORTED;
+  {
+    cudaError_t ce = cudaFuncSetAttribute(head_loss_bwd_kernel, cudaFuncAttributeMaxDynamicSharedMemorySize, (int)c.smem);
+    if (ce == cudaSuccess)
+      ce = cudaFuncSetAttribute(head_loss_bwd_kernel, cudaFuncAttributePreferredSharedMemoryCarveout,
+                                cudaSharedmemCarveoutMaxShared);
+    if (ce != cudaSuccess) return (int)ce;
+  }
+  head_loss_bwd_kernel<<<grid, 32 * c.nw, c.smem, st>>>(h);
+  rb::count_launch();
+  {
+    cudaError_t ce = cudaPeekAtLastError();
+    if (ce != cudaSuccess) return (int)ce;
+  }
+  if ((e = rb200_ppo_loss(ppo, stream))) return e;
+  return head_grads_and_towers(L, P, wsplit, states, idx, n, h.part, grid, a.with_critic != 0, acts, work, grads, st);
 }
 
 extern "C" int rb200_mlp_sample(const rb200_mlp_layout* L, const float* params, const float* wsplit,
diff --git a/rlinf_b200/ops.py b/rlinf_b200/ops.py
--- a/rlinf_b200/ops.py
+++ b/rlinf_b200/ops.py
@@ -91,13 +91,11 @@
     return out
 
 
-def ppo_loss(*, logprobs, old_logprobs, advantages, C_chunks, A_dim, logprob_type, values=None, returns=None,
-             prev_values=None, loss_mask=None, loss_mask_sum=None, mask_sum_row_mod=0, idx=None, entropy=None,
-             adv_stats=None, adv_norm_eps=1e-5, clip_ratio_low=0.2, clip_ratio_high=0.2, clip_ratio_c=None,
-             clip_log_ratio_min=None, clip_log_ratio_max=None, value_clip=0.0, huber_delta=0.0,
-             max_episode_steps=None, critic_warmup=False, entropy_bonus=0.0, loss_scale=1.0, want_grads=True,
-             _decoupled=None):
-    lib = L.load()
+def _ppo_args(*, logprobs, old_logprobs, advantages, C_chunks, A_dim, logprob_type, values=None, returns=None,
+              prev_values=None, loss_mask=None, loss_mask_sum=None, mask_sum_row_mod=0, idx=None, entropy=None,
+              adv_stats=None, adv_norm_eps=1e-5, clip_ratio_low=0.2, clip_ratio_high=0.2, clip_ratio_c=None,
+              clip_log_ratio_min=None, clip_log_ratio_max=None, value_clip=0.0, huber_delta=0.0,
+              max_episode_steps=None, critic_warmup=False, entropy_bonus=0.0, loss_scale=1.0, want_grads=True):
     dev = logprobs.device
     bsz = logprobs.shape[0]
     with_critic = values is not None
@@ -150,6 +148,32 @@
     d_e = torch.empty_like(keep[0]) if (want_grads and entropy is not None) else None
     a.workspace, a.loss, a.metrics = L.ptr(ws), L.ptr(loss), L.ptr(metrics)
     a.d_logprobs, a.d_values, a.d_entropy = L.ptr(d_lp), L.ptr(d_v), L.ptr(d_e)
+    return a, keep, loss, metrics, d_lp, d_v, d_e
+
+
+def ppo_loss(*, logprobs, old_logprobs, advantages, C_chunks, A_dim, logprob_type, values=None, returns=None,
+             prev_values=None, loss_mask=None, loss_mask_sum=None, mask_sum_row_mod=0, idx=None, entropy=None,
+             adv_stats=None, adv_norm_eps=1e-5, clip_ratio_low=0.2, clip_ratio_high=0.2, clip_ratio_c=None,
+             clip_log_ratio_min=None, clip_log_ratio_max=None, value_clip=0.0, huber_delta=0.0,
+             max_episode_steps=None, critic_warmup=False, entropy_bonus=0.0, loss_scale=1.0, want_grads=True,
+             _decoupled=None):
+    lib = L.load()
+    a, keep, loss, metrics, d_lp, d_v, d_e = _ppo_args(
+        logprobs=logprobs, old_logprobs=old_logprobs, advantages=advantages, C_chunks=C_chunks, A_dim=A_dim,
+        logprob_type=logprob_type, values=values, returns=returns, prev_values=prev_values, loss_mask=loss_mask,
+        loss_mask_sum=loss_mask_sum, mask_sum_row_mod=mask_sum_row_mod, idx=idx, entropy=entropy, adv_stats=adv_stats,
+        adv_norm_eps=adv_norm_eps, clip_ratio_low=clip_ratio_low, clip_ratio_high=clip_ratio_high,
+        clip_ratio_c=clip_ratio_c, clip_log_ratio_min=clip_log_ratio_min, clip_log_ratio_max=clip_log_ratio_max,
+        value_clip=value_clip, huber_delta=huber_delta, max_episode_steps=max_episode_steps,
+        critic_warmup=critic_warmup, entropy_bonus=entropy_bonus, loss_scale=loss_scale, want_grads=want_grads)
+
+    def P(t, dtype=None):
+        if t is None:
+            return None
+        t = L.to_device(t, logprobs.device, dtype)
+        keep.append(t)
+        return L.ptr(t)
+
     if _decoupled is not None and _decoupled.get("version") is not None:
         if _decoupled.get("versions") is not None or _decoupled.get("current_version") is None:
             raise ValueError("a scalar `version` needs `current_version` and excludes the `versions` tensor")
diff --git a/rlinf_b200/policy.py b/rlinf_b200/policy.py
--- a/rlinf_b200/policy.py
+++ b/rlinf_b200/policy.py
@@ -147,6 +147,32 @@
             out["values"] = vals
         return out
 
+    def forward_loss_backward(self, states, action, compute_entropy=True, compute_values=True, states_amax=None,
+                              **ppo):
+        from . import ops
+
+        lib = L.load()
+        n = states.shape[0]
+        logp = torch.empty((n, self.act_dim), dtype=torch.float32, device=self.device)
+        ent = torch.empty_like(logp) if compute_entropy else None
+        vals = torch.empty((n, self.value_dim), dtype=torch.float32, device=self.device) if (
+            compute_values and self.value_dim > 0) else None
+        a, keep, loss, metrics, *_ = ops._ppo_args(logprobs=logp, values=vals, entropy=ent, want_grads=False, **ppo)
+        if not lib.rb200_mlp_head_loss_supported(C.byref(self.layout), C.byref(a)):
+            return None
+        nscr = lib.rb200_mlp_fwd_scratch_floats(C.byref(self.layout), n)
+        acts = self._buf("acts", nscr)
+        work = self._buf("work", nscr)
+        L.check(lib.rb200_mlp_forward_towers(C.byref(self.layout), L.ptr(self.flat_params), self._ws(), L.ptr(states),
+                                             None, n, int(vals is not None), L.ptr(acts), L.ptr(states_amax),
+                                             L.stream_ptr()), "mlp_forward_towers")
+        L.check(lib.rb200_mlp_head_loss_backward(C.byref(self.layout), L.ptr(self.flat_params), self._ws(),
+                                                 L.ptr(states), L.ptr(action), None, n, C.byref(a), L.ptr(acts),
+                                                 L.ptr(work), L.ptr(self.flat_grads), L.stream_ptr()),
+                "mlp_head_loss_backward")
+        self._last = (states, action, None, n, acts)
+        return loss, metrics
+
     def backward(self, d_logprobs, d_values=None, d_entropy=None):
         lib = L.load()
         states, action, idx, n, acts = self._last
```

Result: faster. 6.776 million, median of 6 (+2.5%).
